# lgen-sudo/EgoM2P

Measured on NVIDIA B200. Metric: ego-b mod4 train nominal tokens/sec (whole job), higher is better.
Workload: dtype bf16

## Files before the change

### egom2p_b200/_lib.py

```python
from __future__ import annotations

import ctypes as C
import os

_HERE = os.path.dirname(os.path.abspath(__file__))
LIB_PATH = os.path.join(_HERE, "libegom2p_b200.so")
MAX_MODS = 8

vp, i32, i64, f32 = C.c_void_p, C.c_int32, C.c_int64, C.c_float


class PlanDesc(C.Structure):
    _fields_ = [("n_mods", i32), ("batch", i32), ("budget", i32), ("is_decoder", i32), ("causal", i32), ("sep", i32),
                ("len", i32 * MAX_MODS), ("mod_id", i32 * MAX_MODS), ("mask", vp * MAX_MODS),
                ("attn_cnt", vp * MAX_MODS), ("ids", vp * MAX_MODS)]


class EmbedDesc(C.Structure):
    _fields_ = [("n_mods", i32), ("dim", i32), ("len", i32 * MAX_MODS), ("vocab", i32 * MAX_MODS),
                ("ids", vp * MAX_MODS), ("token_emb", vp * MAX_MODS), ("pos_emb", vp * MAX_MODS),
                ("mod_emb", vp * MAX_MODS)]


SIGNATURES = {
    "egom2p_last_error": [],
    "egom2p_abi_version": [],
    "egom2p_launch_count": [],
    "egom2p_index_plan": [C.POINTER(PlanDesc), vp, vp, vp, vp, vp, vp, vp, vp, vp, vp],
    "egom2p_plan_rows": [vp, i64, C.POINTER(i32), i32, i64, vp, vp, vp],
    "egom2p_embed_gather_fwd": [C.POINTER(EmbedDesc), vp, vp, vp, vp, vp, i64, i32, vp, vp, vp],
    "egom2p_embed_gather_bwd": [C.POINTER(EmbedDesc), vp, vp, vp, vp, vp, vp, i64, i32, vp, vp, vp, vp],
    "egom2p_layernorm_fwd": [vp, vp, i64, i32, f32, vp, vp, vp, vp, vp],
    "egom2p_layernorm_bwd": [vp, vp, vp, vp, vp, vp, vp, i64, i32, vp, vp, vp, vp],
    "egom2p_layernorm_bias_fwd": [vp, vp, vp, i64, i32, f32, vp, vp, vp, vp, vp],
    "egom2p_layernorm_bias_bwd": [vp, vp, vp, vp, vp, vp, vp, i64, i32, vp, vp, vp, vp, vp],
    "egom2p_gemm_bf16": [vp, vp, i32, i32, i32, i64, i64, i32, i32, vp, vp, i64, vp, vp, i64, vp],
    "egom2p_gemm_swiglu_fwd": [vp, vp, i32, i32, i32, i64, i64, vp, i64, vp, i64, vp],
    "egom2p_gemm_swiglu_bwd": [vp, vp, vp, i32, i32, i32, i64, i64, i64, vp, i64, vp],
    "egom2p_gemm_gelu_fwd": [vp, vp, vp, i32, i32, i32, i64, i64, vp, i64, vp, i64, vp],
    "egom2p_gemm_gelu_bwd": [vp, vp, vp, i32, i32, i32, i64, i64, i64, vp, i64, vp],
    "egom2p_ce_partials": [vp, vp, vp, i32, i32, i32, i64, i64, vp, vp, vp, vp],
    "egom2p_ce_finalize": [vp, vp, vp, i32, i32, vp, vp, vp],
    "egom2p_ce_dlogits": [vp, vp, vp, vp, vp, i32, i32, i32, i32, i64, i64, vp, i64, vp],
    "egom2p_attn_lse_stride": [i32],
    "egom2p_attn_ranges_bytes": [i32, i32],
    "egom2p_attn_ranges": [vp, vp, i32, i32, i32, f32, i32, vp, vp],
    "egom2p_attn_fwd": [vp, vp, vp, i32, i32, i32, i32, i64, i64, i64, vp, vp, i64, vp, vp, vp],
    "egom2p_attn_bwd_scratch_bytes": [i32, i32, i32],
    "egom2p_attn_bwd": [vp, vp, vp, vp, vp, vp, i32, i32, i32, i32, i64, i64, i64, i64, vp, f32, vp, vp, vp, vp,
                        i64, i64, i64, vp],
    "egom2p_cast_f32_to_bf16": [vp, vp, i64, vp],
    "egom2p_cast_f32_to_bf16_multi": [vp, i32, i64, vp],
    "egom2p_add_f32": [vp, vp, i64, vp, vp, vp],
    "egom2p_sumsq_multi": [vp, i32, i64, vp, vp, vp],
    "egom2p_adamw_multi_steps": [vp, i32, i64, f32, f32, f32, vp, vp, f32, vp],
    "egom2p_image_masks": [vp, C.c_uint64, C.c_uint64, i32, i32, i32, vp, vp, vp, vp, vp, vp],
    "egom2p_sample_rows": [vp, i64, i32, i32, f32, f32, i32, vp, vp, vp, vp, vp],
    "egom2p_cfg_combine_bf16": [vp, vp, i64, f32, vp, vp],
    "egom2p_colsum_f32": [vp, i64, i32, vp, vp],
    "egom2p_colsum_bf16": [vp, i64, i32, i64, vp, vp],
    "egom2p_gather_rows_bf16": [vp, vp, i64, i32, vp, vp],
    "egom2p_scatter_rows_f32": [vp, vp, i64, i32, vp, vp],
}
_RESTYPES = {"egom2p_last_error": C.c_char_p, "egom2p_launch_count": i64, "egom2p_attn_bwd_scratch_bytes": i64, "egom2p_attn_ranges_bytes": i64}

_lib = None


def load() -> C.CDLL:
    global _lib
    if _lib is None:
        if not os.path.exists(LIB_PATH):
            raise RuntimeError(f"{LIB_PATH} not found: the CUDA library is mandatory (no fallback path). "
                               "Run `python -m egom2p_b200.build`.")
        lib = C.CDLL(LIB_PATH)
        for name, args in SIGNATURES.items():
            fn = getattr(lib, name)
            fn.argtypes = args
            fn.restype = _RESTYPES.get(name, C.c_int)
        _lib = lib
    return _lib


def check(rc: int, what: str = "") -> None:
    if rc != 0:
        msg = load().egom2p_last_error()
        raise RuntimeError(f"egom2p_b200 {what} failed (code {rc}): {msg.decode() if msg else '?'}")


def launch_count() -> int:
    return int(load().egom2p_launch_count())
```

### egom2p_b200/csrc/attn_bwd.cu

```cuda
#include "attn_common.cuh"

namespace egom2p {

constexpr int kBwdMathWarps = 8;
constexpr int kBwdThreads = 32 * (kBwdMathWarps + 7);
constexpr int kDrainWarp0 = kBwdMathWarps, kBwdTmaWarp = kBwdMathWarps + 4, kBwdMmaWarp = kBwdMathWarps + 5,
              kBwdMmaWarpB = kBwdMathWarps + 6;
constexpr int kBwdStages = 3;
constexpr int kBwdMetaBytes = 5 * kT * 4;
constexpr int kMaxQBlocks = 1024;

struct BwdParams {
  int B, H, Mq, Nk, S;
  RangeMeta meta;
  const float* lse2;
  const float* ndelta;
  float scale_log2;
  uint16_t* dK;
  uint16_t* dV;
  int64_t lddk, lddv;
  int tma_out;
};
struct BwdSmem {
  static constexpr int kTile = kT * 128;
  static constexpr int kK = 0, kV = kK + kTile, kQ = kV + kTile, kDO = kQ + kBwdStages * kTile,
                       kDS = kDO + kBwdStages * kTile,
                       kBox = kDS + 2 * kTile,
                       kMeta = kBox + 8 * 4096, kList = kMeta + kBwdStages * kBwdMetaBytes,
                       kBar = kList + kMaxQBlocks * 2, kTotal = kBar + 256 + 1024;
};
static_assert(BwdSmem::kTotal <= 232448, "attention backward exceeds the 227 KB shared memory of one CTA");


#ifdef EGOM2P_TRACE
__device__ long long g_trace[16 * 64];
#define TRACE(slot, idx)                                                                          \
  do {                                                                                            \
    if (blockIdx.x == 0 && blockIdx.y == 0 && blockIdx.z == gridDim.z - 1 && (idx) < 64 && (threadIdx.x & 31) == 0) \
      g_trace[(slot) * 64 + (idx)] = clock64();                                                   \
  } while (0)
#else
#define TRACE(slot, idx) do {} while (0)
#endif

__device__ __forceinline__ void tmem_st32(uint32_t taddr, const uint32_t (&r)[32]) {
  asm volatile(
      "tcgen05.st.sync.aligned.32x32b.x32.b32 [%0], "
      "{%1, %2, %3, %4, %5, %6, %7, %8, %9, %10, %11, %12, %13, %14, %15, %16, "
      "%17, %18, %19, %20, %21, %22, %23, %24, %25, %26, %27, %28, %29, %30, %31, %32};"
      ::"r"(taddr), "r"(r[0]), "r"(r[1]), "r"(r[2]), "r"(r[3]), "r"(r[4]), "r"(r[5]), "r"(r[6]), "r"(r[7]), "r"(r[8]),
        "r"(r[9]), "r"(r[10]), "r"(r[11]), "r"(r[12]), "r"(r[13]), "r"(r[14]), "r"(r[15]), "r"(r[16]), "r"(r[17]),
        "r"(r[18]), "r"(r[19]), "r"(r[20]), "r"(r[21]), "r"(r[22]), "r"(r[23]), "r"(r[24]), "r"(r[25]), "r"(r[26]),
        "r"(r[27]), "r"(r[28]), "r"(r[29]), "r"(r[30]), "r"(r[31])
      : "memory");
}
__device__ __forceinline__ void tmem_st16(uint32_t taddr, const uint32_t (&r)[16]) {
  asm volatile(
      "tcgen05.st.sync.aligned.32x32b.x16.b32 [%0], "
      "{%1, %2, %3, %4, %5, %6, %7, %8, %9, %10, %11, %12, %13, %14, %15, %16};"
      ::"r"(taddr), "r"(r[0]), "r"(r[1]), "r"(r[2]), "r"(r[3]), "r"(r[4]), "r"(r[5]), "r"(r[6]), "r"(r[7]), "r"(r[8]),
        "r"(r[9]), "r"(r[10]), "r"(r[11]), "r"(r[12]), "r"(r[13]), "r"(r[14]), "r"(r[15])
      : "memory");
}
__device__ __forceinline__ void tmem_st_wait() { asm volatile("tcgen05.wait::st.sync.aligned;" ::: "memory"); }
__device__ __forceinline__ float4 lds_f4(const void* p) {
  float4 v;
  asm volatile("ld.shared.v4.f32 {%0, %1, %2, %3}, [%4];" : "=f"(v.x), "=f"(v.y), "=f"(v.z), "=f"(v.w) : "r"(smem_u32(p)));
  return v;
}

__global__ void __launch_bounds__(kBwdThreads, 1)
attn_bwd_kernel(const __grid_constant__ CUtensorMap tmQ, const __grid_constant__ CUtensorMap tmDO,
                const __grid_constant__ CUtensorMap tmK, const __grid_constant__ CUtensorMap tmV,
                const __grid_constant__ CUtensorMap tmDQ, const __grid_constant__ CUtensorMap tmDK,
                const __grid_constant__ CUtensorMap tmDV, const BwdParams p) {
  extern __shared__ uint8_t smem_raw[];
  uint8_t* smem = reinterpret_cast<uint8_t*>((reinterpret_cast<uintptr_t>(smem_raw) + 1023) & ~(uintptr_t)1023);
  uint8_t *sK = smem + BwdSmem::kK, *sV = smem + BwdSmem::kV, *sQ = smem + BwdSmem::kQ, *sDO = smem + BwdSmem::kDO,
          *sDS = smem + BwdSmem::kDS, *sBox = smem + BwdSmem::kBox, *sMeta = smem + BwdSmem::kMeta;
  uint16_t* s_list = reinterpret_cast<uint16_t*>(smem + BwdSmem::kList);
  uint64_t* bars = reinterpret_cast<uint64_t*>(smem + BwdSmem::kBar);
  uint64_t* kv_full = bars;
  uint64_t* q_full = bars + 1;
  uint64_t* q_empty = q_full + kBwdStages;
  uint64_t* s_full = q_empty + kBwdStages;
  uint64_t* s_free = s_full + 1;
  uint64_t* dp_full = s_free + 1;
  uint64_t* dp_free = dp_full + 1;
  uint64_t* p_full = dp_free + 1;
  uint64_t* p_empty = p_full + 1;
  uint64_t* ds_full = p_empty + 1;
  uint64_t* ds_empty = ds_full + 1;
  uint64_t* dq_full = ds_empty + 1;
  uint64_t* dq_free = dq_full + 1;
  uint64_t* dkv_full = dq_free + 1;
  uint64_t* kv_tmem = dkv_full + 1;
  uint32_t* tmem_slot = reinterpret_cast<uint32_t*>(kv_tmem + 1);
  int* s_n = reinterpret_cast<int*>(tmem_slot + 1);

  const int warp = threadIdx.x >> 5, lane = threadIdx.x & 31;
  const int kv0 = blockIdx.x * kT, h = blockIdx.y, b = blockIdx.z;
  const int nqb = p.S / kT;
  if (warp == 0) TRACE(5, 63);
  if (warp == kDrainWarp0 && lane == 0) {
    tma_prefetch_desc(&tmQ);
    tma_prefetch_desc(&tmDO);
    tma_prefetch_desc(&tmDQ);
    tma_prefetch_desc(&tmDK);
    tma_prefetch_desc(&tmDV);
  }
  if (warp == kBwdTmaWarp && lane == 0) {
    mbar_init(kv_full, 1);
    fence_mbar_init();
    mbar_expect_tx(kv_full, 2 * BwdSmem::kTile);
    tma_load_2d(sK, &tmK, kv_full, h * kD, b * p.Nk + kv0);
    tma_load_2d(sV, &tmV, kv_full, h * kD, b * p.Nk + kv0);
    for (int i = 0; i < kBwdStages; ++i) { mbar_init(&q_full[i], 1); mbar_init(&q_empty[i], 1); }
    mbar_init(s_full, 1);   mbar_init(s_free, kBwdMathWarps);
    mbar_init(dp_full, 1);  mbar_init(dp_free, 1);
    mbar_init(p_full, kBwdMathWarps);  mbar_init(p_empty, 1);
    mbar_init(ds_full, kBwdMathWarps); mbar_init(ds_empty, 1);
    mbar_init(dq_full, 1);  mbar_init(dq_free, 4);
    mbar_init(dkv_full, 1);
    mbar_init(kv_tmem, kBwdMathWarps);
    fence_mbar_init();
    TRACE(5, 57);
  }
  auto issue_q_block = [&](int qblk, int st) {
    const int r0 = qblk * kT;
    uint8_t* meta = sMeta + st * kBwdMetaBytes;
    const int64_t hoff = ((int64_t)b * p.H + h) * p.S + r0, roff = (int64_t)b * p.S + r0;
    mbar_expect_tx(&q_full[st], 2 * BwdSmem::kTile + kBwdMetaBytes);
    tma_load_2d(sQ + st * BwdSmem::kTile, &tmQ, &q_full[st], h * kD, b * p.Mq + r0);
    tma_load_2d(sDO + st * BwdSmem::kTile, &tmDO, &q_full[st], h * kD, b * p.Mq + r0);
    bulk_load(meta + 0 * 512, p.lse2 + hoff, 512, &q_full[st]);
    bulk_load(meta + 1 * 512, p.ndelta + hoff, 512, &q_full[st]);
    bulk_load(meta + 2 * 512, p.meta.row_lo + roff, 512, &q_full[st]);
    bulk_load(meta + 3 * 512, p.meta.row_hi + roff, 512, &q_full[st]);
    bulk_load(meta + 4 * 512, p.meta.row_scale + roff, 512, &q_full[st]);
  };
  if (warp == kBwdTmaWarp) {
    int first = -1;
    for (int i0 = 0; i0 < nqb && first < 0; i0 += 32) {
      const int i = i0 + lane;
      bool take = false;
      if (i < nqb) {
        const int64_t o = ((int64_t)b * nqb + i) * 2;
        const int lo = min(p.meta.blk_lo[o], p.meta.blk_lo[o + 1]), hi = max(p.meta.blk_hi[o], p.meta.blk_hi[o + 1]);
        take = hi > kv0 && lo < kv0 + kT;
      }
      const unsigned msk = __ballot_sync(0xffffffffu, take);
      if (msk) first = i0 + __ffs(msk) - 1;
    }
    __syncwarp();
    if (first >= 0 && lane == 0) issue_q_block(first, 0);
  }
  if (warp == 0) {
    int n = 0;
    for (int i0 = 0; i0 < nqb; i0 += 32) {
      const int i = i0 + lane;
      bool take = false, inside = false, normal = false;
      if (i < nqb) {
        const int64_t o = ((int64_t)b * nqb + i) * 2;
        const int lo = min(p.meta.blk_lo[o], p.meta.blk_lo[o + 1]), hi = max(p.meta.blk_hi[o], p.meta.blk_hi[o + 1]);
        take = hi > kv0 && lo < kv0 + kT;
        inside = max(p.meta.blk_lo_max[o], p.meta.blk_lo_max[o + 1]) <= kv0 &&
                 min(p.meta.blk_hi_min[o], p.meta.blk_hi_min[o + 1]) >= kv0 + kT;
        normal = p.meta.blk_lo_max[o] != INT_MAX && p.meta.blk_lo_max[o + 1] != INT_MAX;
      }
      const unsigned msk = __ballot_sync(0xffffffffu, take);
      const int pos = n + __popc(msk & ((1u << lane) - 1));
      if (take && pos < kMaxQBlocks) s_list[pos] = (uint16_t)(i | (inside ? 0x8000 : 0) | (normal ? 0x4000 : 0));
      n += __popc(msk);
    }
    if (lane == 0) *s_n = n < kMaxQBlocks ? n : kMaxQBlocks;
    TRACE(5, 55);
  }
  if (warp == kBwdMmaWarp) {
    tmem_alloc<512>(tmem_slot);
    TRACE(5, 54);
  }
  if (warp == 1) TRACE(5, 53);
  tc_fence_before();
  __syncthreads();
  tc_fence_after();
  const uint32_t tmem_base = *tmem_slot;
  const int n = *s_n;
  if (warp == 0) TRACE(5, 62);
  constexpr uint32_t cS = 0, cDP = 128, cDV = 256, cDK = 320, cDQ = 384, cK = 448, cV = 480;

  if (warp >= kBwdTmaWarp) {
    if (warp == kBwdTmaWarp) {
      if (n == 0) mbar_wait(kv_full, 0);
      if (n > 0) {
        for (int idx = 1; idx < n; ++idx) {
          const int st = idx % kBwdStages;
          mbar_wait(&q_empty[st], ((idx / kBwdStages) & 1) ^ 1);
          if (elect_one()) issue_q_block((int)(s_list[idx] & 0x3fff), st);
          __syncwarp();
        }
      }
    } else if (warp == kBwdMmaWarp) {
      if (n > 0) {
        constexpr uint32_t idesc_kk = umma_idesc_bf16(128, kT, 0, 0);
        constexpr uint32_t idesc_tm = umma_idesc_bf16(128, kD, 0, 1);
        constexpr uint32_t idesc_mm = umma_idesc_bf16(128, kD, 1, 1);
        const uint32_t tS = tmem_base + cS, tDP = tmem_base + cDP, tDQ = tmem_base + cDQ, tK = tmem_base + cK, tV = tmem_base + cV;
        const uint64_t dKm0 = umma_desc_mnmajor_sw128(smem_u32(sK), 8192);
        const uint64_t dDSm0 = umma_desc_mnmajor_sw128(smem_u32(sDS), BwdSmem::kTile);
        auto issue_s = [&](int st) {
          const uint64_t dQ0 = umma_desc_kmajor_sw128(smem_u32(sQ + st * BwdSmem::kTile));
          if (elect_one()) {
#pragma unroll
            for (int k = 0; k < 4; ++k) umma_bf16_ts(tS, tK + 8 * k, dQ0 + 2 * k, idesc_kk, k ? 1u : 0u);
            umma_commit(s_full);
          }
          __syncwarp();
        };
        auto issue_dp = [&](int st) {
          const uint64_t dDO0 = umma_desc_kmajor_sw128(smem_u32(sDO + st * BwdSmem::kTile));
          if (elect_one()) {
#pragma unroll
            for (int k = 0; k < 4; ++k) umma_bf16_ts(tDP, tV + 8 * k, dDO0 + 2 * k, idesc_kk, k ? 1u : 0u);
            umma_commit(dp_full);
          }
          __syncwarp();
        };
        mbar_wait(kv_tmem, 0);
        mbar_wait(&q_full[0], 0);
        tc_fence_after();
        issue_s(0);
        issue_dp(0);
        for (int idx = 0; idx < n; ++idx) {
          const int st1 = (idx + 1) % kBwdStages;
          const uint32_t par = idx & 1;
          if (idx + 1 < n) {
            mbar_wait(&q_full[st1], ((idx + 1) / kBwdStages) & 1);
            mbar_wait(s_free, par);
            mbar_wait(p_empty, par);
            tc_fence_after();
            TRACE(0, idx);
            issue_s(st1);
          }
          mbar_wait(ds_full, par);
          if (idx > 0) mbar_wait(dq_free, (idx - 1) & 1);
          tc_fence_after();
          TRACE(4, idx);
          if (elect_one()) {
#pragma unroll
            for (int k = 0; k < 8; ++k) umma_bf16_ss(tDQ, dDSm0 + 128 * k, dKm0 + 128 * k, idesc_mm, k ? 1u : 0u);
            umma_commit(dq_full);
            umma_commit(ds_empty);
          }
          __syncwarp();
          if (idx + 1 < n) {
            mbar_wait(dp_free, par);
            tc_fence_after();
            TRACE(2, idx);
            issue_dp(st1);
          }
        }
      }
    } else if (warp == kBwdMmaWarpB) {
      if (n > 0) {
        constexpr uint32_t idesc_tm = umma_idesc_bf16(128, kD, 0, 1);
        const uint32_t tS = tmem_base + cS, tDP = tmem_base + cDP, tDV = tmem_base + cDV, tDK = tmem_base + cDK;
        for (int idx = 0; idx < n; ++idx) {
          const int st = idx % kBwdStages;
          const uint32_t par = idx & 1;
          mbar_wait(p_full, par);
          tc_fence_after();
          TRACE(1, idx);
          const uint64_t dDOm0 = umma_desc_mnmajor_sw128(smem_u32(sDO + st * BwdSmem::kTile), 8192);
          if (elect_one()) {
#pragma unroll
            for (int k = 0; k < 8; ++k)
              umma_bf16_ts(tDV, tS + (k < 4 ? 8 * k : 64 + 8 * (k - 4)), dDOm0 + 128 * k, idesc_tm, (idx | k) ? 1u : 0u);
            umma_commit(p_empty);
          }
          __syncwarp();
          mbar_wait(ds_full, par);
          tc_fence_after();
          TRACE(3, idx);
          const uint64_t dQm0 = umma_desc_mnmajor_sw128(smem_u32(sQ + st * BwdSmem::kTile), 8192);
          if (elect_one()) {
#pragma unroll
            for (int k = 0; k < 8; ++k)
              umma_bf16_ts(tDK, tDP + (k < 4 ? 8 * k : 64 + 8 * (k - 4)), dQm0 + 128 * k, idesc_tm, (idx | k) ? 1u : 0u);
            umma_commit(&q_empty[st]);
            umma_commit(dp_free);
            if (idx == n - 1) umma_commit(dkv_full);
          }
          __syncwarp();
        }
      }
    }
  } else if (warp >= kDrainWarp0) {
    const int quarter = warp & 3;
    uint8_t* box0 = sBox + quarter * 8192;
    const uint32_t t_dq = tmem_base + ((uint32_t)(quarter * 32) << 16) + cDQ;
    for (int idx = 0; idx < n; ++idx) {
      const int r0 = (int)(s_list[idx] & 0x3fff) * kT + quarter * 32;
      mbar_wait(dq_full, idx & 1);
      tc_fence_after();
      if (warp == kDrainWarp0) TRACE(11, idx);
      const bool live = r0 < p.Mq;
      if (lane == 0) tma_store_wait_read();
      __syncwarp();
#pragma unroll
      for (int hb = 0; hb < 2; ++hb) {
        uint32_t v[32];
        uint8_t* box = box0 + hb * 4096;
        tmem_ld32(t_dq + hb * 32, v);
        tmem_ld_wait();
        if (hb == 1) {
          tc_fence_before();
          __syncwarp();
          if (lane == 0) mbar_arrive(dq_free);
        }
        if (live) {
#pragma unroll
          for (int j = 0; j < 8; ++j)
            *reinterpret_cast<uint4*>(box + lane * 128 + ((j ^ (lane & 7)) << 4)) = make_uint4(v[4 * j], v[4 * j + 1], v[4 * j + 2], v[4 * j + 3]);
          fence_async_smem();
          __syncwarp();
          if (lane == 0) {
            tma_reduce_add_2d(&tmDQ, box, h * kD + hb * 32, b * p.Mq + r0);
            tma_store_commit();
          }
        }
      }
      if (warp == kDrainWarp0) TRACE(12, idx);
    }
    if (lane == 0) tma_store_wait_read();
  } else {
    const int quarter = warp & 3, half = warp >> 2;
    const int trow = quarter * 32 + lane;
    const int kidx = kv0 + trow;
    const uint32_t t_lane = tmem_base + ((uint32_t)(quarter * 32) << 16);
    uint8_t* pDS = sDS + half * BwdSmem::kTile;
    const float SC = p.scale_log2, RN = p.scale_log2 * kLn2;
    if (n > 0) {
      mbar_wait(kv_full, 0);
      if (warp == 0) TRACE(5, 56);
      uint32_t kw[16], vw[16];
#pragma unroll
      for (int c = 0; c < 4; ++c) {
        const uint4 a = *reinterpret_cast<const uint4*>(sK + swz_off(trow, half * 4 + c));
        const uint4 d = *reinterpret_cast<const uint4*>(sV + swz_off(trow, half * 4 + c));
        kw[4 * c] = a.x; kw[4 * c + 1] = a.y; kw[4 * c + 2] = a.z; kw[4 * c + 3] = a.w;
        vw[4 * c] = d.x; vw[4 * c + 1] = d.y; vw[4 * c + 2] = d.z; vw[4 * c + 3] = d.w;
      }
      tmem_st16(t_lane + cK + half * 16, kw);
      tmem_st16(t_lane + cV + half * 16, vw);
      tmem_st_wait();
      tc_fence_before();
      __syncwarp();
      if (lane == 0) mbar_arrive(kv_tmem);
      if (warp == 0) TRACE(5, 58);
    }
    for (int idx = 0; idx < n; ++idx) {
      const int st = idx % kBwdStages;
      const uint32_t par = idx & 1;
      const bool inside = (s_list[idx] & 0x8000) != 0, normal = (s_list[idx] & 0x4000) != 0;
      const float* m_ls = reinterpret_cast<const float*>(sMeta + st * kBwdMetaBytes) + half * 64;
      const float* m_nd = m_ls + kT;
      const int* m_lo = reinterpret_cast<const int*>(m_ls + 2 * kT);
      const int* m_hi = m_lo + kT;
      const float* m_rs = m_ls + 4 * kT;
      uint32_t pp[32];
      {
        uint32_t s0[32], s1[32];
        if (warp == 0) TRACE(5, idx);
        mbar_wait(&q_full[st], (idx / kBwdStages) & 1);
        mbar_wait(s_full, par);
        tc_fence_after();
        if (warp == 0) TRACE(6, idx);
        tmem_ld32(t_lane + cS + half * 64, s0);
        tmem_ld32(t_lane + cS + half * 64 + 32, s1);
        tmem_ld_wait();
        tc_fence_before();
        __syncwarp();
        if (lane == 0) mbar_arrive(s_free);
        if (inside) {
#pragma unroll
          for (int c4 = 0; c4 < 8; ++c4) {
            const float4 la = lds_f4(m_ls + 4 * c4), lb = lds_f4(m_ls + 32 + 4 * c4);
            s0[4 * c4] = __float_as_uint(fmaf(__uint_as_float(s0[4 * c4]), SC, -la.x));
            s0[4 * c4 + 1] = __float_as_uint(fmaf(__uint_as_float(s0[4 * c4 + 1]), SC, -la.y));
            s0[4 * c4 + 2] = __float_as_uint(fmaf(__uint_as_float(s0[4 * c4 + 2]), SC, -la.z));
            s0[4 * c4 + 3] = __float_as_uint(fmaf(__uint_as_float(s0[4 * c4 + 3]), SC, -la.w));
            s1[4 * c4] = __float_as_uint(fmaf(__uint_as_float(s1[4 * c4]), SC, -lb.x));
            s1[4 * c4 + 1] = __float_as_uint(fmaf(__uint_as_float(s1[4 * c4 + 1]), SC, -lb.y));
            s1[4 * c4 + 2] = __float_as_uint(fmaf(__uint_as_float(s1[4 * c4 + 2]), SC, -lb.z));
            s1[4 * c4 + 3] = __float_as_uint(fmaf(__uint_as_float(s1[4 * c4 + 3]), SC, -lb.w));
          }
#pragma unroll
          for (int c = 0; c < 32; ++c) {
            s0[c] = __float_as_uint((c & 3) == 3 ? ex2_poly(__uint_as_float(s0[c])) : ex2(__uint_as_float(s0[c])));
            s1[c] = __float_as_uint((c & 3) == 3 ? ex2_poly(__uint_as_float(s1[c])) : ex2(__uint_as_float(s1[c])));
          }
#pragma unroll
          for (int c = 0; c < 16; ++c) {
            pp[c] = pack_bf16(__uint_as_float(s0[2 * c]), __uint_as_float(s0[2 * c + 1]));
            pp[16 + c] = pack_bf16(__uint_as_float(s1[2 * c]), __uint_as_float(s1[2 * c + 1]));
          }
        } else if (normal) {
#pragma unroll
          for (int c4 = 0; c4 < 8; ++c4) {
#pragma unroll
            for (int g = 0; g < 2; ++g) {
              uint32_t(&sv)[32] = g ? s1 : s0;
              const float4 l = lds_f4(m_ls + g * 32 + 4 * c4), lo = lds_f4(m_lo + g * 32 + 4 * c4), hi = lds_f4(m_hi + g * 32 + 4 * c4);
              const float lv[4] = {l.x, l.y, l.z, l.w};
              const int lov[4] = {__float_as_int(lo.x), __float_as_int(lo.y), __float_as_int(lo.z), __float_as_int(lo.w)};
              const int hiv[4] = {__float_as_int(hi.x), __float_as_int(hi.y), __float_as_int(hi.z), __float_as_int(hi.w)};
#pragma unroll
              for (int u = 0; u < 4; ++u) {
                const bool ok = kidx >= lov[u] && kidx < hiv[u];
                sv[4 * c4 + u] = ok ? __float_as_uint(fmaf(__uint_as_float(sv[4 * c4 + u]), SC, -lv[u])) : 0xff800000u;
              }
            }
          }
#pragma unroll
          for (int c = 0; c < 32; ++c) {
            s0[c] = __float_as_uint(ex2(__uint_as_float(s0[c])));
            s1[c] = __float_as_uint(ex2(__uint_as_float(s1[c])));
          }
#pragma unroll
          for (int c = 0; c < 16; ++c) {
            pp[c] = pack_bf16(__uint_as_float(s0[2 * c]), __uint_as_float(s0[2 * c + 1]));
            pp[16 + c] = pack_bf16(__uint_as_float(s1[2 * c]), __uint_as_float(s1[2 * c + 1]));
          }
        } else {
#pragma unroll
          for (int c = 0; c < 32; ++c) {
            float e[2];
#pragma unroll
            for (int u = 0; u < 2; ++u) {
              const int q = 2 * c + u;
              const float rs = m_rs[q];
              const bool ok = kidx >= m_lo[q] && kidx < m_hi[q];
              const float sv = __uint_as_float(q < 32 ? s0[q & 31] : s1[q & 31]);
              e[u] = ok ? ex2(fmaf(rs != 0.f ? sv : 0.f, rs, -m_ls[q])) : 0.f;
            }
            pp[c] = pack_bf16(e[0], e[1]);
          }
        }
      }
      if (warp == 0) TRACE(7, idx);
      tmem_st32(t_lane + cS + half * 64, pp);
      uint32_t d0[32];
      mbar_wait(dp_full, par);
      tc_fence_after();
      tmem_ld32(t_lane + cDP + half * 64, d0);
      tmem_st_wait();
      tc_fence_before();
      __syncwarp();
      if (lane == 0) mbar_arrive(p_full);
      if (warp == 0) TRACE(8, idx);
      auto dsmul = [&](const uint32_t (&d)[32], int hh) {
        if (inside || normal) {
#pragma unroll
          for (int c4 = 0; c4 < 8; ++c4) {
            const float4 nd = lds_f4(m_nd + hh * 32 + 4 * c4);
            const uint32_t t0 = pack_bf16(fmaf(__uint_as_float(d[4 * c4]), RN, nd.x), fmaf(__uint_as_float(d[4 * c4 + 1]), RN, nd.y));
            const uint32_t t1 = pack_bf16(fmaf(__uint_as_float(d[4 * c4 + 2]), RN, nd.z), fmaf(__uint_as_float(d[4 * c4 + 3]), RN, nd.w));
            asm("mul.rn.bf16x2 %0, %1, %2;" : "=r"(pp[hh * 16 + 2 * c4]) : "r"(pp[hh * 16 + 2 * c4]), "r"(t0));
            asm("mul.rn.bf16x2 %0, %1, %2;" : "=r"(pp[hh * 16 + 2 * c4 + 1]) : "r"(pp[hh * 16 + 2 * c4 + 1]), "r"(t1));
          }
        } else {
#pragma unroll
          for (int c4 = 0; c4 < 8; ++c4) {
            const float4 nd = lds_f4(m_nd + hh * 32 + 4 * c4);
            const float4 rs = lds_f4(m_rs + hh * 32 + 4 * c4);
            const uint32_t t0 = pack_bf16(fmaf(__uint_as_float(d[4 * c4]), rs.x * kLn2, nd.x), fmaf(__uint_as_float(d[4 * c4 + 1]), rs.y * kLn2, nd.y));
            const uint32_t t1 = pack_bf16(fmaf(__uint_as_float(d[4 * c4 + 2]), rs.z * kLn2, nd.z), fmaf(__uint_as_float(d[4 * c4 + 3]), rs.w * kLn2, nd.w));
            asm("mul.rn.bf16x2 %0, %1, %2;" : "=r"(pp[hh * 16 + 2 * c4]) : "r"(pp[hh * 16 + 2 * c4]), "r"(t0));
            asm("mul.rn.bf16x2 %0, %1, %2;" : "=r"(pp[hh * 16 + 2 * c4 + 1]) : "r"(pp[hh * 16 + 2 * c4 + 1]), "r"(t1));
          }
        }
      };
      tmem_ld_wait();
      if (warp == 0) TRACE(9, idx);
      dsmul(d0, 0);
      if (warp == 0) TRACE(13, idx);
      tmem_ld32(t_lane + cDP + half * 64 + 32, d0);
      if (idx > 0) mbar_wait(ds_empty, (idx - 1) & 1);
      tmem_ld_wait();
      if (warp == 0) TRACE(14, idx);
      dsmul(d0, 1);
      if (warp == 0) TRACE(15, idx);
      tmem_st32(t_lane + cDP + half * 64, pp);
#pragma unroll
      for (int c8 = 0; c8 < 8; ++c8)
        *reinterpret_cast<uint4*>(pDS + swz_off(trow, c8)) = make_uint4(pp[4 * c8], pp[4 * c8 + 1], pp[4 * c8 + 2], pp[4 * c8 + 3]);
      fence_async_smem();
      tmem_st_wait();
      tc_fence_before();
      __syncwarp();
      if (lane == 0) mbar_arrive(ds_full);
      if (warp == 0) TRACE(10, idx);
    }
    if (n > 0) {
      mbar_wait(dkv_full, 0);
      tc_fence_after();
    }
    if (warp == 0) TRACE(5, 61);
#pragma unroll 1
    for (int which = 0; which < 2; ++which) {
      uint32_t v[32];
      if (n > 0) {
        tmem_ld32(t_lane + (which == 0 ? cDV : cDK) + half * 32, v);
        tmem_ld_wait();
      } else {
#pragma unroll
        for (int c = 0; c < 32; ++c) v[c] = 0u;
      }
      uint4 pk[4];
#pragma unroll
      for (int c8 = 0; c8 < 4; ++c8) {
        pk[c8].x = pack_bf16(__uint_as_float(v[c8 * 8 + 0]), __uint_as_float(v[c8 * 8 + 1]));
        pk[c8].y = pack_bf16(__uint_as_float(v[c8 * 8 + 2]), __uint_as_float(v[c8 * 8 + 3]));
        pk[c8].z = pack_bf16(__uint_as_float(v[c8 * 8 + 4]), __uint_as_float(v[c8 * 8 + 5]));
        pk[c8].w = pack_bf16(__uint_as_float(v[c8 * 8 + 6]), __uint_as_float(v[c8 * 8 + 7]));
      }
      if (p.tma_out) {
        uint8_t* stage = which == 0 ? sQ : sDO;
#pragma unroll
        for (int c8 = 0; c8 < 4; ++c8) *reinterpret_cast<uint4*>(stage + swz_off(trow, half * 4 + c8)) = pk[c8];
        if (warp == 0) TRACE(5, 52 - which);
      } else if (kidx < p.Nk) {
        uint16_t* out = (which == 0 ? p.dV + ((int64_t)b * p.Nk + kidx) * p.lddv : p.dK + ((int64_t)b * p.Nk + kidx) * p.lddk) +
                        h * kD + half * 32;
#pragma unroll
        for (int c8 = 0; c8 < 4; ++c8) reinterpret_cast<uint4*>(out)[c8] = pk[c8];
      }
    }
    if (p.tma_out) {
      fence_async_smem();
      asm volatile("bar.sync 1, 256;" ::: "memory");
      if (warp == 0) TRACE(5, 50);
      if (warp == 0 && lane == 0) {
        tma_store_2d(&tmDV, sQ, h * kD, b * p.Nk + kv0);
        tma_store_2d(&tmDK, sDO, h * kD, b * p.Nk + kv0);
        tma_store_commit();
        tma_store_wait_read();
      }
    }
    if (warp == 0) TRACE(5, 60);
  }
  tc_fence_before();
  __syncthreads();
  if (warp == 0) TRACE(5, 59);
  if (warp == kBwdMmaWarp) {
    tc_fence_after();
    tmem_dealloc<512>(tmem_base);
  }
}

__global__ void __launch_bounds__(256) attn_bwd_prep_kernel(const uint16_t* __restrict__ O, const uint16_t* __restrict__ dO,
                                                            int64_t ldo, const float* __restrict__ row_scale, int B, int H,
                                                            int Mq, int S, float* __restrict__ ndelta, float* __restrict__ dq_acc) {
  const int64_t wid = (int64_t)blockIdx.x * 8 + (threadIdx.x >> 5);
  const int lane = threadIdx.x & 31;
  if (wid >= (int64_t)B * S) return;
  const int b = (int)(wid / S), r = (int)(wid % S);
  if (r >= Mq) {
    for (int hh = lane; hh < H; hh += 32) ndelta[((int64_t)b * H + hh) * S + r] = 0.f;
    return;
  }
  const float rs = row_scale[wid] * kLn2;
  const uint16_t* po = O + ((int64_t)b * Mq + r) * ldo;
  const uint16_t* pd = dO + ((int64_t)b * Mq + r) * ldo;
  float4* acc = reinterpret_cast<float4*>(dq_acc + ((int64_t)b * Mq + r) * (int64_t)H * kD);
  const int chunks = H * 8;
  for (int c0 = 0; c0 < chunks; c0 += 32) {
    const int c = c0 + lane;
    float part = 0.f;
    if (c < chunks) {
      const uint4 a = reinterpret_cast<const uint4*>(po)[c], g = reinterpret_cast<const uint4*>(pd)[c];
      const uint32_t aw[4] = {a.x, a.y, a.z, a.w}, gw[4] = {g.x, g.y, g.z, g.w};
#pragma unroll
      for (int u = 0; u < 4; ++u) {
        const float2 fa = __bfloat1622float2(*reinterpret_cast<const __nv_bfloat162*>(&aw[u]));
        const float2 fg = __bfloat1622float2(*reinterpret_cast<const __nv_bfloat162*>(&gw[u]));
        part += fa.x * fg.x + fa.y * fg.y;
      }
      acc[2 * c] = make_float4(0.f, 0.f, 0.f, 0.f);
      acc[2 * c + 1] = make_float4(0.f, 0.f, 0.f, 0.f);
    }
    part += __shfl_xor_sync(0xffffffffu, part, 1);
    part += __shfl_xor_sync(0xffffffffu, part, 2);
    part += __shfl_xor_sync(0xffffffffu, part, 4);
    if (c < chunks && (lane & 7) == 0) ndelta[((int64_t)b * H + (c >> 3)) * S + r] = -part * rs;
  }
}

__global__ void __launch_bounds__(256) attn_bwd_dq_cast_kernel(const float* __restrict__ acc, int64_t rows, int cols8,
                                                               uint16_t* __restrict__ dq, int64_t lddq) {
  const int64_t total = rows * cols8;
  for (int64_t i = (int64_t)blockIdx.x * blockDim.x + threadIdx.x; i < total; i += (int64_t)gridDim.x * blockDim.x) {
    const int64_t r = i / cols8;
    const int c = (int)(i % cols8);
    const float4 a = reinterpret_cast<const float4*>(acc + r * cols8 * 8)[2 * c];
    const float4 g = reinterpret_cast<const float4*>(acc + r * cols8 * 8)[2 * c + 1];
    uint4 pk;
    pk.x = pack_bf16(a.x, a.y); pk.y = pack_bf16(a.z, a.w); pk.z = pack_bf16(g.x, g.y); pk.w = pack_bf16(g.z, g.w);
    reinterpret_cast<uint4*>(dq + r * lddq)[c] = pk;
  }
}

}

#ifdef EGOM2P_TRACE
extern "C" int egom2p_debug_attn_trace(long long* host_dst) {
  return (int)cudaMemcpyFromSymbol(host_dst, egom2p::g_trace, sizeof(egom2p::g_trace));
}
#endif

extern "C" int64_t egom2p_attn_bwd_scratch_bytes(int32_t B, int32_t H, int32_t Mq) {
  using namespace egom2p;
  return align256((int64_t)B * H * padS(Mq) * 4) + align256((int64_t)B * Mq * H * kD * 4) + 256;
}

extern "C" int egom2p_attn_bwd(const uint16_t* Q, const uint16_t* K, const uint16_t* V, const uint16_t* O, const uint16_t* dO,
                               const float* lse, int32_t B, int32_t H, int32_t Mq, int32_t Nk, int64_t ldq, int64_t ldk,
                               int64_t ldv, int64_t ldo, const void* meta, float scale, void* scratch, uint16_t* dQ,
                               uint16_t* dK, uint16_t* dV, int64_t lddq, int64_t lddk, int64_t lddv, void* stream_) {
  using namespace egom2p;
  cudaStream_t stream = (cudaStream_t)stream_;
  EGO_REQUIRE(Q && O && dO && lse && meta && scratch && dQ && B > 0 && H > 0 && Mq > 0 && Nk >= 0, "attn_bwd: bad argument");
  EGO_REQUIRE(((uintptr_t)scratch & 255) == 0 && ((uintptr_t)lse & 255) == 0 && ((uintptr_t)meta & 255) == 0,
              "attn_bwd: scratch / lse / meta must be 256-byte aligned");
  EGO_REQUIRE(lddq % 8 == 0 && ((uintptr_t)dQ & 15) == 0 && ldo % 8 == 0 && ((uintptr_t)O & 15) == 0 && ((uintptr_t)dO & 15) == 0,
              "attn_bwd: dQ / O / dO alignment");
  const int S = padS(Mq);
  EGO_REQUIRE(S / kT <= kMaxQBlocks, "attn_bwd: Mq too large (max %d)", kMaxQBlocks * kT);
  RangeMeta rm = carve_meta(const_cast<void*>(meta), B, Mq);
  float* ndelta = reinterpret_cast<float*>(scratch);
  float* dq_acc = reinterpret_cast<float*>(reinterpret_cast<char*>(scratch) + align256((int64_t)B * H * S * 4));

  attn_bwd_prep_kernel<<<(unsigned)(((int64_t)B * S + 7) / 8), 256, 0, stream>>>(O, dO, ldo, rm.row_scale, B, H, Mq, S, ndelta, dq_acc);
  int rc = check_launch("attn_bwd prep");
  if (rc) return rc;
  if (Nk > 0) {
    EGO_REQUIRE(K && V && dK && dV, "attn_bwd: K / V / dK / dV missing");
    EGO_REQUIRE(lddk % 8 == 0 && lddv % 8 == 0 && ((uintptr_t)dK & 15) == 0 && ((uintptr_t)dV & 15) == 0, "attn_bwd: dK/dV alignment");
    static std::atomic<uint64_t> attr_done{0};
    if ((rc = ensure_dyn_smem(attn_bwd_kernel, BwdSmem::kTotal, attr_done, "attn_bwd"))) return rc;
    CUtensorMap tmQ, tmDO, tmK, tmV, tmDQ, tmDK, tmDV;
    if ((rc = make_tmap_bf16_2d(&tmQ, Q, (uint64_t)B * Mq, (uint64_t)H * kD, ldq, kT, kD))) return rc;
    if ((rc = make_tmap_bf16_2d(&tmDO, dO, (uint64_t)B * Mq, (uint64_t)H * kD, ldo, kT, kD))) return rc;
    if ((rc = make_tmap_bf16_2d(&tmK, K, (uint64_t)B * Nk, (uint64_t)H * kD, ldk, kT, kD))) return rc;
    if ((rc = make_tmap_bf16_2d(&tmV, V, (uint64_t)B * Nk, (uint64_t)H * kD, ldv, kT, kD))) return rc;
    if ((rc = make_tmap_2d(&tmDQ, dq_acc, 4, (uint64_t)B * Mq, (uint64_t)H * kD, (uint64_t)H * kD, 32, 32))) return rc;
    const int tma_out = (Nk % kT == 0 || B == 1) ? 1 : 0;
    if (tma_out) {
      if ((rc = make_tmap_bf16_2d(&tmDK, dK, (uint64_t)B * Nk, (uint64_t)H * kD, lddk, kT, kD))) return rc;
      if ((rc = make_tmap_bf16_2d(&tmDV, dV, (uint64_t)B * Nk, (uint64_t)H * kD, lddv, kT, kD))) return rc;
    } else {
      tmDK = tmK;
      tmDV = tmV;
    }
    BwdParams pb{B, H, Mq, Nk, S, rm, lse, ndelta, scale * kLog2e, dK, dV, lddk, lddv, tma_out};
    attn_bwd_kernel<<<dim3((Nk + kT - 1) / kT, H, B), kBwdThreads, BwdSmem::kTotal, stream>>>(tmQ, tmDO, tmK, tmV, tmDQ, tmDK, tmDV, pb);
    if ((rc = check_launch("attn_bwd"))) return rc;
  }
  const int64_t rows = (int64_t)B * Mq;
  const int cols8 = H * kD / 8;
  const int64_t total = rows * cols8;
  attn_bwd_dq_cast_kernel<<<(unsigned)((total + 255) / 256 < 148 * 16 ? (total + 255) / 256 : 148 * 16), 256, 0, stream>>>(dq_acc, rows, cols8, dQ, lddq);
  return check_launch("attn_bwd dq cast");
}
```

### egom2p_b200/ops.py

```python
from __future__ import annotations

import ctypes as C
from typing import Dict, Optional, Sequence

import torch

from . import _lib

bf16, f32 = torch.bfloat16, torch.float32


def _s() -> int:
    return torch.cuda.current_stream().cuda_stream


def _req_current(t: torch.Tensor):
    if t.device.index is not None and t.device.index != torch.cuda.current_device():
        raise RuntimeError(f"egom2p_b200: tensor on {t.device} but the current CUDA device is {torch.cuda.current_device()}; "
                           "wrap the call in torch.cuda.device(tensor.device)")


class KernelTimer:
    active: Optional["KernelTimer"] = None

    def __init__(self):
        self.records = []

    def __enter__(self):
        KernelTimer.active = self
        return self

    def __exit__(self, *exc):
        KernelTimer.active = None

    def summary(self):
        torch.cuda.synchronize()
        out: Dict[str, Dict[str, float]] = {}
        for fam, work, unit, e0, e1 in self.records:
            d = out.setdefault(fam, {"ms": 0.0, "work": 0.0, "launches": 0, "unit": unit})
            d["ms"] += e0.elapsed_time(e1)
            d["work"] += float(work)
            d["launches"] += 1
        return out


class _timed:
    __slots__ = ("fam", "work", "unit", "e0")

    def __init__(self, fam: str, work: float, unit: str):
        self.fam, self.work, self.unit = fam, work, unit

    def __enter__(self):
        if KernelTimer.active is not None:
            self.e0 = torch.cuda.Event(enable_timing=True)
            self.e0.record()

    def __exit__(self, *exc):
        t = KernelTimer.active
        if t is not None:
            e1 = torch.cuda.Event(enable_timing=True)
            e1.record()
            t.records.append((self.fam, self.work, self.unit, self.e0, e1))


def _p(t: Optional[torch.Tensor]):
    return None if t is None else t.data_ptr()


def _req(t: torch.Tensor, dtype, name: str):
    if not t.is_cuda:
        raise RuntimeError(f"egom2p_b200: {name} must be a CUDA tensor (no CPU fallback exists)")
    if t.dtype != dtype:
        raise TypeError(f"egom2p_b200: {name} must be {dtype}, got {t.dtype}")
    _req_current(t)
    return t


class Plan:
    __slots__ = ("keep_idx", "keep_mod", "keep_pos", "pad", "mod_mask", "n_valid", "target_ids", "key_lo", "key_hi",
                 "B", "budget", "order", "row_batch", "rows", "slot_index", "slot_to_row")

    def __init__(self):
        self.row_batch = None
        self.rows = None


def index_plan(masks: Sequence[torch.Tensor], mod_ids: Sequence[int], budget: int, *, decoder: bool = False,
               attn_cnt: Optional[Sequence[torch.Tensor]] = None, ids: Optional[Sequence[torch.Tensor]] = None,
               causal: bool = False, sep: bool = True) -> Plan:
    lib = _lib.load()
    B = masks[0].shape[0]
    dev = masks[0].device
    d = _lib.PlanDesc()
    d.n_mods, d.batch, d.is_decoder, d.causal, d.sep = len(masks), B, int(decoder), int(causal), int(sep)
    keep = []
    total = 0
    for i, m in enumerate(masks):
        m = _req(m.reshape(B, -1), torch.bool, "mask").contiguous()
        keep.append(m)
        d.len[i], d.mod_id[i], d.mask[i] = m.shape[1], int(mod_ids[i]), m.data_ptr()
        total += m.shape[1]
        if decoder:
            a = _req(attn_cnt[i].reshape(B, -1), torch.int32, "decoder_attention_mask").contiguous()
            t = _req(ids[i].reshape(B, -1), torch.int64, "ids").contiguous()
            keep += [a, t]
            d.attn_cnt[i], d.ids[i] = a.data_ptr(), t.data_ptr()
    budget = min(int(budget), total)
    d.budget = budget
    pl = Plan()
    pl.B, pl.budget = B, budget
    pl.keep_idx = torch.empty(B, budget, dtype=torch.int32, device=dev)
    pl.keep_mod = torch.empty_like(pl.keep_idx)
    pl.keep_pos = torch.empty_like(pl.keep_idx)
    pl.pad = torch.empty(B, budget, dtype=torch.bool, device=dev)
    pl.mod_mask = torch.empty(B, budget, dtype=torch.int16, device=dev)
    pl.n_valid = torch.empty(B, dtype=torch.int32, device=dev)
    pl.target_ids = pl.key_lo = pl.key_hi = None
    if decoder:
        pl.target_ids = torch.empty(B, budget, dtype=torch.int64, device=dev)
        pl.key_lo = torch.empty(B, budget, dtype=torch.int32, device=dev)
        pl.key_hi = torch.empty_like(pl.key_lo)
    _lib.check(lib.egom2p_index_plan(C.byref(d), _p(pl.keep_idx), _p(pl.keep_mod), _p(pl.keep_pos), _p(pl.pad),
                                     _p(pl.mod_mask), _p(pl.n_valid), _p(pl.target_ids), _p(pl.key_lo), _p(pl.key_hi),
                                     _s()), "index_plan")
    return pl


def plan_rows(mod_mask: torch.Tensor, mod_ids: Sequence[int]):
    lib = _lib.load()
    _req(mod_mask, torch.int16, "mod_mask")
    flat = mod_mask.reshape(-1).contiguous()
    total, n = flat.numel(), len(mod_ids)
    rows = torch.empty(n, total, dtype=torch.int64, device=flat.device)
    counts = torch.empty(n, dtype=torch.int32, device=flat.device)
    ids = (C.c_int32 * n)(*[int(i) for i in mod_ids])
    _lib.check(lib.egom2p_plan_rows(_p(flat), total, ids, n, total, _p(rows), _p(counts), _s()), "plan_rows")
    return rows, counts


def _embed_desc(dim, lens, vocabs, ids, tables, pos, mod):
    d = _lib.EmbedDesc()
    d.n_mods, d.dim = len(lens), dim
    for i in range(len(lens)):
        d.len[i], d.vocab[i] = lens[i], vocabs[i]
        d.ids[i] = _p(ids[i]) if ids is not None else None
        d.token_emb[i] = _p(tables[i]) if tables is not None else None
        d.pos_emb[i], d.mod_emb[i] = _p(pos[i]), _p(mod[i])
    return d


def embed_gather_fwd(plan: Plan, dim: int, lens, vocabs, ids, tables, pos, mod, mask_token=None, want_emb=True):
    lib = _lib.load()
    packed = plan.rows is not None
    rows = plan.rows if packed else plan.B * plan.budget
    dev = plan.keep_mod.device
    x0 = torch.empty((rows, dim) if packed else (plan.B, plan.budget, dim), dtype=f32, device=dev)
    emb = torch.empty_like(x0) if want_emb else None
    d = _embed_desc(dim, lens, vocabs, ids, tables, pos, mod)
    with _timed("embed_gather", rows * dim * 4.0 * (2 + (1 if mask_token is None else 0) + (1 if want_emb else 0)), "byte"):
        _lib.check(lib.egom2p_embed_gather_fwd(C.byref(d), _p(mask_token), _p(plan.keep_mod), _p(plan.keep_pos), _p(plan.pad),
                                               _p(plan.row_batch), rows, plan.budget, _p(x0), _p(emb), _s()), "embed_gather_fwd")
    return x0, emb


def embed_gather_bwd(plan: Plan, dim: int, lens, vocabs, ids, pos, mod, dx0, demb, d_tables, d_mod, d_mask_token):
    lib = _lib.load()
    rows = plan.rows if plan.rows is not None else plan.B * plan.budget
    d = _embed_desc(dim, lens, vocabs, ids, None, pos, mod)
    n = len(lens)
    arr_t = (C.c_void_p * _lib.MAX_MODS)(*[(_p(t) if t is not None else None) for t in (d_tables or [None] * n)])
    arr_m = (C.c_void_p * _lib.MAX_MODS)(*[(_p(t) if t is not None else None) for t in (d_mod or [None] * n)])
    _lib.check(lib.egom2p_embed_gather_bwd(C.byref(d), _p(dx0), _p(demb), _p(plan.keep_mod), _p(plan.keep_pos),
                                           _p(plan.pad), _p(plan.row_batch), rows, plan.budget, C.cast(arr_t, C.c_void_p),
                                           C.cast(arr_m, C.c_void_p), _p(d_mask_token), _s()), "embed_gather_bwd")


def layernorm_fwd(x: torch.Tensor, w: torch.Tensor, eps: float = 1e-6, out_bf16=True, out_f32=False, save_stats=True, bias=None):
    lib = _lib.load()
    _req(x, f32, "x"); _req(w, f32, "weight")
    D = x.shape[-1]
    rows = x.numel() // D
    yb = torch.empty(x.shape, dtype=bf16, device=x.device) if out_bf16 else None
    yf = torch.empty_like(x) if out_f32 else None
    mean = torch.empty(rows, dtype=f32, device=x.device) if save_stats else None
    rstd = torch.empty(rows, dtype=f32, device=x.device) if save_stats else None
    with _timed("layernorm_fwd", rows * D * (4.0 + (2 if out_bf16 else 0) + (4 if out_f32 else 0)), "byte"):
        if bias is None:
            _lib.check(lib.egom2p_layernorm_fwd(_p(x), _p(w), rows, D, eps, _p(yb), _p(yf), _p(mean), _p(rstd), _s()), "layernorm_fwd")
        else:
            _req(bias, f32, "bias")
            _lib.check(lib.egom2p_layernorm_bias_fwd(_p(x), _p(w), _p(bias), rows, D, eps, _p(yb), _p(yf), _p(mean), _p(rstd), _s()),
                       "layernorm_bias_fwd")
    return yb, yf, mean, rstd


def layernorm_bwd(dy: torch.Tensor, x, w, mean, rstd, dx_in=None, d_weight=None, want_bf16=False, d_bias=None):
    lib = _lib.load()
    D = x.shape[-1]
    rows = x.numel() // D
    dx = torch.empty_like(x)
    dxb = torch.empty(x.shape, dtype=bf16, device=x.device) if want_bf16 else None
    dyb = dy if dy.dtype == bf16 else None
    dyf = dy if dy.dtype == f32 else None
    nbytes = rows * D * (4.0 + dy.element_size() + 4 + (4 if dx_in is not None else 0) + (2 if want_bf16 else 0))
    with _timed("layernorm_bwd", nbytes, "byte"):
        if d_bias is None:
            _lib.check(lib.egom2p_layernorm_bwd(_p(dyb), _p(dyf), _p(x), _p(w), _p(mean), _p(rstd), _p(dx_in), rows, D, _p(dx),
                                                _p(dxb), _p(d_weight), _s()), "layernorm_bwd")
        else:
            _req(d_bias, f32, "d_bias")
            _lib.check(lib.egom2p_layernorm_bias_bwd(_p(dyb), _p(dyf), _p(x), _p(w), _p(mean), _p(rstd), _p(dx_in), rows, D,
                                                     _p(dx), _p(dxb), _p(d_weight), _p(d_bias), _s()), "layernorm_bias_bwd")
    return dx, dxb


def gemm(A: torch.Tensor, B: torch.Tensor, M: int, N: int, K: int, *, a_mn=False, b_mn=False, bias=None, addend=None,
         out_bf16: Optional[torch.Tensor] = None, out_f32: Optional[torch.Tensor] = None):
    lib = _lib.load()
    _req(A, bf16, "A"); _req(B, bf16, "B")
    assert A.dim() == 2 and B.dim() == 2 and A.stride(1) == 1 and B.stride(1) == 1
    out = out_bf16 if out_bf16 is not None else out_f32
    assert out is not None and out.stride(-1) == 1
    ldc = out.stride(0)
    if out_bf16 is not None and out_f32 is not None:
        assert out_bf16.stride(0) == out_f32.stride(0)
    with _timed("gemm", 2.0 * M * N * K, "flop"):
        _lib.check(lib.egom2p_gemm_bf16(_p(A), _p(B), M, N, K, A.stride(0), B.stride(0), int(a_mn), int(b_mn), _p(bias),
                                        _p(addend), addend.stride(0) if addend is not None else 0, _p(out_bf16), _p(out_f32),
                                        ldc, _s()), "gemm_bf16")
    return out


def gemm_swiglu_fwd(x: torch.Tensor, w13: torch.Tensor):
    lib = _lib.load()
    R, K = x.shape
    N2 = w13.shape[0]
    ab = torch.empty(R, N2, dtype=bf16, device=x.device)
    g = torch.empty(R, N2 // 2, dtype=bf16, device=x.device)
    with _timed("gemm", 2.0 * R * N2 * K, "flop"):
        _lib.check(lib.egom2p_gemm_swiglu_fwd(_p(x), _p(w13), R, N2, K, x.stride(0), w13.stride(0), _p(ab), ab.stride(0), _p(g),
                                              g.stride(0), _s()), "gemm_swiglu_fwd")
    return ab, g


def gemm_swiglu_bwd(dy: torch.Tensor, w2: torch.Tensor, ab: torch.Tensor):
    lib = _lib.load()
    R, K = dy.shape
    hidden = w2.shape[1]
    dab = torch.empty(R, 2 * hidden, dtype=bf16, device=dy.device)
    with _timed("gemm", 2.0 * R * hidden * K, "flop"):
        _lib.check(lib.egom2p_gemm_swiglu_bwd(_p(dy), _p(w2), _p(ab), R, hidden, K, dy.stride(0), w2.stride(0), ab.stride(0),
                                              _p(dab), dab.stride(0), _s()), "gemm_swiglu_bwd")
    return dab


def gemm_gelu_fwd(x: torch.Tensor, w1: torch.Tensor, b1: Optional[torch.Tensor]):
    lib = _lib.load()
    R, K = x.shape
    N = w1.shape[0]
    if b1 is not None:
        _req(b1, f32, "b1")
    u = torch.empty(R, N, dtype=bf16, device=x.device)
    h = torch.empty(R, N, dtype=bf16, device=x.device)
    with _timed("gemm", 2.0 * R * N * K, "flop"):
        _lib.check(lib.egom2p_gemm_gelu_fwd(_p(x), _p(w1), _p(b1), R, N, K, x.stride(0), w1.stride(0), _p(u), u.stride(0), _p(h),
                                            h.stride(0), _s()), "gemm_gelu_fwd")
    return u, h


def gemm_gelu_bwd(dy: torch.Tensor, w2: torch.Tensor, u: torch.Tensor):
    lib = _lib.load()
    R, K = dy.shape
    hidden = w2.shape[1]
    du = torch.empty(R, hidden, dtype=bf16, device=dy.device)
    with _timed("gemm", 2.0 * R * hidden * K, "flop"):
        _lib.check(lib.egom2p_gemm_gelu_bwd(_p(dy), _p(w2), _p(u), R, hidden, K, dy.stride(0), w2.stride(0), u.stride(0), _p(du),
                                            du.stride(0), _s()), "gemm_gelu_bwd")
    return du


def linear_fwd(x: torch.Tensor, w: torch.Tensor, *, bias=None, addend=None, out_dtype=bf16):
    R, K = x.shape
    N = w.shape[0]
    y = torch.empty(R, N, dtype=out_dtype, device=x.device)
    gemm(x, w, R, N, K, bias=bias, addend=addend, out_bf16=y if out_dtype == bf16 else None,
         out_f32=y if out_dtype == f32 else None)
    return y


def linear_dgrad(dy: torch.Tensor, w: torch.Tensor, *, addend=None, out_dtype=bf16):
    R, N = dy.shape
    K = w.shape[1]
    dx = torch.empty(R, K, dtype=out_dtype, device=dy.device)
    gemm(dy, w, R, K, N, b_mn=True, addend=addend, out_bf16=dx if out_dtype == bf16 else None,
         out_f32=dx if out_dtype == f32 else None)
    return dx


def linear_wgrad(dy: torch.Tensor, x: torch.Tensor, out: Optional[torch.Tensor] = None, accumulate=False):
    R, N = dy.shape
    K = x.shape[1]
    if out is None:
        out = torch.empty(N, K, dtype=f32, device=dy.device)
    gemm(dy, x, N, K, R, a_mn=True, b_mn=True, addend=out if accumulate else None, out_f32=out)
    return out


def ce_forward(y: torch.Tensor, w: torch.Tensor, target: torch.Tensor):
    lib = _lib.load()
    R, K = y.shape
    V = w.shape[0]
    nt = 2 * ((V + 255) // 256)
    dev = y.device
    pm = torch.empty(nt, R, dtype=f32, device=dev)
    ps = torch.empty(nt, R, dtype=f32, device=dev)
    tl = torch.zeros(R, dtype=f32, device=dev)
    lse = torch.empty(R, dtype=f32, device=dev)
    loss = torch.zeros(1, dtype=f32, device=dev)
    with _timed("head_ce", 2.0 * R * V * K, "flop"):
        _lib.check(lib.egom2p_ce_partials(_p(y), _p(w), _p(target), R, V, K, y.stride(0), w.stride(0), _p(pm), _p(ps), _p(tl),
                                          _s()), "ce_partials")
    _lib.check(lib.egom2p_ce_finalize(_p(pm), _p(ps), _p(tl), R, nt, _p(lse), _p(loss), _s()), "ce_finalize")
    return loss, lse


def ce_dlogits(y, w, target, lse, gscale: torch.Tensor, v0: int, vc: int, out: torch.Tensor):
    lib = _lib.load()
    R, K = y.shape
    with _timed("head_ce", 2.0 * R * vc * K, "flop"):
        _lib.check(lib.egom2p_ce_dlogits(_p(y), _p(w), _p(target), _p(lse), _p(gscale), R, v0, vc, K, y.stride(0), w.stride(0),
                                         _p(out), out.stride(0), _s()), "ce_dlogits")
    return out


def lse_stride(Mq: int) -> int:
    return int(_lib.load().egom2p_attn_lse_stride(Mq))


def attn_ranges(B, Mq, Nk, key_lo=None, key_hi=None, scale=None, device=None, empty_zero=False):
    lib = _lib.load()
    scale = (64 ** -0.5) if scale is None else scale
    device = device if device is not None else key_lo.device
    meta = torch.empty(lib.egom2p_attn_ranges_bytes(B, Mq), dtype=torch.uint8, device=device)
    _lib.check(lib.egom2p_attn_ranges(_p(key_lo), _p(key_hi), B, Mq, Nk, scale, int(empty_zero), _p(meta), _s()), "attn_ranges")
    return meta


def attn_fwd(q, k, v, B, H, Mq, Nk, key_lo=None, key_hi=None, scale=None, want_lse=True, meta=None, pairs=None):
    lib = _lib.load()
    if meta is None:
        meta = attn_ranges(B, Mq, Nk, key_lo, key_hi, scale, device=q.device)
    o = torch.empty(B * Mq, H * 64, dtype=bf16, device=q.device)
    lse = torch.empty(B, H, lse_stride(Mq), dtype=f32, device=q.device) if want_lse else None
    kmax = torch.empty(B * H, dtype=f32, device=q.device) if Nk > 0 else None
    with _timed("attn_fwd", 4.0 * H * 64 * (pairs if pairs is not None else B * Mq * Nk), "flop"):
        _lib.check(lib.egom2p_attn_fwd(_p(q), _p(k) if Nk > 0 else None, _p(v) if Nk > 0 else None, B, H, Mq, Nk, q.stride(0),
                                       k.stride(0) if Nk > 0 else 0, v.stride(0) if Nk > 0 else 0, _p(meta), _p(o),
                                       o.stride(0), _p(lse), _p(kmax), _s()), "attn_fwd")
    return o, lse


def attn_bwd(q, k, v, o, do, lse, B, H, Mq, Nk, dq, dk, dv, key_lo=None, key_hi=None, scale=None, meta=None, pairs=None):
    lib = _lib.load()
    scale = (64 ** -0.5) if scale is None else scale
    if meta is None:
        meta = attn_ranges(B, Mq, Nk, key_lo, key_hi, scale, device=q.device)
    assert do.stride(0) == o.stride(0)
    scratch = torch.empty(lib.egom2p_attn_bwd_scratch_bytes(B, H, Mq), dtype=torch.uint8, device=q.device)
    with _timed("attn_bwd", 10.0 * H * 64 * (pairs if pairs is not None else B * Mq * Nk), "flop"):
        _lib.check(lib.egom2p_attn_bwd(_p(q), _p(k), _p(v), _p(o), _p(do), _p(lse), B, H, Mq, Nk, q.stride(0), k.stride(0),
                                       v.stride(0), o.stride(0), _p(meta), scale, _p(scratch), _p(dq), _p(dk), _p(dv),
                                       dq.stride(0), dk.stride(0), dv.stride(0), _s()), "attn_bwd")


def cast_bf16(src: torch.Tensor, out: Optional[torch.Tensor] = None):
    lib = _lib.load()
    _req(src, f32, "src")
    src = src.contiguous()
    if out is None:
        out = torch.empty(src.shape, dtype=bf16, device=src.device)
    with _timed("cast", src.numel() * 6.0, "byte"):
        _lib.check(lib.egom2p_cast_f32_to_bf16(_p(src), _p(out), src.numel(), _s()), "cast_f32_to_bf16")
    return out


GRAD_GEN = [0]
_OPERAND_CACHE: Dict[int, tuple] = {}


def cached_bf16(weight: torch.Tensor) -> torch.Tensor:
    w = weight.detach()
    key = id(weight)
    sig = (w.data_ptr(), weight._version, GRAD_GEN[0], tuple(w.shape))
    hit = _OPERAND_CACHE.get(key)
    if hit is not None and hit[0] == sig:
        return hit[1]
    wb = cast_bf16(w.contiguous())
    if len(_OPERAND_CACHE) > 64:
        _OPERAND_CACHE.clear()
    _OPERAND_CACHE[key] = (sig, wb)
    return wb


class CastPlan:

    def __init__(self, items):
        import numpy as np
        dt = np.dtype([("src", "<u8"), ("dst", "<u8"), ("rows", "<i8"), ("first_chunk", "<i8"), ("cols", "<i4"), ("dst_ld", "<i4"),
                       ("group", "<i4"), ("slot", "<i4"), ("rows_per_chunk", "<i4"), ("pad", "<i4")])
        assert dt.itemsize == 56
        tab = np.zeros(len(items), dtype=dt)
        chunk = 0
        self.bytes = 0.0
        self.ptrs = []
        for i, (src, dst, group, slot) in enumerate(items):
            _req(src, f32, "src"); _req(dst, bf16, "dst")
            assert src.dim() == 2 and src.is_contiguous() and dst.dim() == 2 and dst.stride(1) == 1
            rows, cols = src.shape
            need_rows = rows if group == 0 else (rows + group - 1) // group * 2 * group
            assert dst.shape[0] >= need_rows and dst.shape[1] >= cols, "cast plan: destination too small"
            rpc = max(1, 8192 // cols)
            tab[i] = (src.data_ptr(), dst.data_ptr(), rows, chunk, cols, dst.stride(0), group, slot, rpc, 0)
            chunk += (rows + rpc - 1) // rpc
            self.bytes += rows * cols * 6.0
            self.ptrs.append((src.data_ptr(), dst.data_ptr()))
        self.n_items, self.n_chunks = len(items), chunk
        self.table = torch.from_numpy(tab.view(np.uint8).reshape(-1).copy()).to(items[0][0].device)

    def run(self):
        lib = _lib.load()
        with _timed("cast", self.bytes, "byte"):
            _lib.check(lib.egom2p_cast_f32_to_bf16_multi(_p(self.table), self.n_items, self.n_chunks, _s()), "cast_f32_to_bf16_multi")


def add_f32(a, b, want_f32=True, want_bf16=False):
    lib = _lib.load()
    out = torch.empty_like(a) if want_f32 else None
    outb = torch.empty(a.shape, dtype=bf16, device=a.device) if want_bf16 else None
    _lib.check(lib.egom2p_add_f32(_p(a), _p(b), a.numel(), _p(out), _p(outb), _s()), "add_f32")
    return out, outb


def colsum(x: torch.Tensor, out: torch.Tensor):
    lib = _lib.load()
    rows, cols = x.shape
    _lib.check(lib.egom2p_colsum_f32(_p(x), rows, cols, _p(out), _s()), "colsum_f32")
    return out


def colsum_bf16(x: torch.Tensor, out: Optional[torch.Tensor] = None):
    lib = _lib.load()
    _req(x, bf16, "x")
    assert x.dim() == 2 and x.stride(1) == 1
    rows, cols = x.shape
    if out is None:
        out = torch.zeros(cols, dtype=f32, device=x.device)
    if rows:
        with _timed("bias_grad", rows * cols * 2.0, "byte"):
            _lib.check(lib.egom2p_colsum_bf16(_p(x), rows, cols, x.stride(0), _p(out), _s()), "colsum_bf16")
    return out


def gather_rows_bf16(src: torch.Tensor, idx: torch.Tensor):
    lib = _lib.load()
    n, cols = idx.numel(), src.shape[1]
    dst = torch.empty(n, cols, dtype=bf16, device=src.device)
    if n:
        _lib.check(lib.egom2p_gather_rows_bf16(_p(src), _p(idx), n, cols, _p(dst), _s()), "gather_rows_bf16")
    return dst


def scatter_rows_f32(src: torch.Tensor, idx: torch.Tensor, dst: torch.Tensor):
    lib = _lib.load()
    n, cols = idx.numel(), src.shape[1]
    if n:
        _lib.check(lib.egom2p_scatter_rows_f32(_p(src), _p(idx), n, cols, _p(dst), _s()), "scatter_rows_f32")
    return dst


def sample_rows(logits: torch.Tensor, temperature: float, top_p: float = 0.0, top_k: int = 0, u: Optional[torch.Tensor] = None,
                want_prob: bool = True, want_kept: bool = False):
    lib = _lib.load()
    _req(logits, f32, "logits")
    assert logits.dim() == 2 and logits.stride(1) == 1
    rows, V = logits.shape
    if u is None:
        u = torch.rand(rows, device=logits.device, dtype=f32)
    _req(u, f32, "u")
    tok = torch.empty(rows, dtype=torch.int64, device=logits.device)
    prob = torch.empty(rows, dtype=f32, device=logits.device) if want_prob else None
    kept = torch.empty(rows, dtype=torch.int32, device=logits.device) if want_kept else None
    if rows:
        with _timed("sample", rows * V * 4.0, "byte"):
            _lib.check(lib.egom2p_sample_rows(_p(logits), logits.stride(0), rows, V, float(temperature), float(top_p), int(top_k),
                                              _p(u.contiguous()), _p(tok), _p(prob), _p(kept), _s()), "sample_rows")
    return tok, prob, kept


def cfg_combine_bf16(y_uncond: torch.Tensor, y_cond: torch.Tensor, scale: float) -> torch.Tensor:
    lib = _lib.load()
    _req(y_uncond, f32, "y_uncond"); _req(y_cond, f32, "y_cond")
    assert y_uncond.shape == y_cond.shape and y_uncond.is_contiguous() and y_cond.is_contiguous()
    out = torch.empty(y_uncond.shape, dtype=bf16, device=y_uncond.device)
    if out.numel():
        _lib.check(lib.egom2p_cfg_combine_bf16(_p(y_uncond), _p(y_cond), y_uncond.numel(), float(scale), _p(out), _s()), "cfg_combine_bf16")
    return out
```

### include/egom2p_b200.h

```cpp
#ifndef EGOM2P_B200_H_
#define EGOM2P_B200_H_
#include <stdint.h>

#ifdef __cplusplus
extern "C" {
#endif

#define EGOM2P_OK 0
#define EGOM2P_ERR_INVALID (-1)
#define EGOM2P_ERR_CUDA (-2)

#define EGOM2P_MAX_MODS 8

const char* egom2p_last_error(void);
int egom2p_abi_version(void);
int64_t egom2p_launch_count(void);

typedef struct {
  int32_t n_mods;
  int32_t batch;
  int32_t budget;
  int32_t is_decoder;
  int32_t causal;
  int32_t sep;
  int32_t len[EGOM2P_MAX_MODS];
  int32_t mod_id[EGOM2P_MAX_MODS];
  const uint8_t* mask[EGOM2P_MAX_MODS];
  const int32_t* attn_cnt[EGOM2P_MAX_MODS];
  const int64_t* ids[EGOM2P_MAX_MODS];
} egom2p_plan_desc;

int egom2p_index_plan(const egom2p_plan_desc* desc, int32_t* keep_idx, int32_t* keep_mod, int32_t* keep_pos,
                      uint8_t* pad, int16_t* mod_mask, int32_t* n_valid, int64_t* target_ids, int32_t* key_lo,
                      int32_t* key_hi, void* stream);

int egom2p_plan_rows(const int16_t* mod_mask, int64_t total, const int32_t* mod_ids, int32_t n_mods, int64_t cap,
                     int64_t* rows, int32_t* counts, void* stream);

typedef struct {
  int32_t n_mods;
  int32_t dim;
  int32_t len[EGOM2P_MAX_MODS];
  int32_t vocab[EGOM2P_MAX_MODS];
  const int64_t* ids[EGOM2P_MAX_MODS];
  const float* token_emb[EGOM2P_MAX_MODS];
  const float* pos_emb[EGOM2P_MAX_MODS];
  const float* mod_emb[EGOM2P_MAX_MODS];
} egom2p_embed_desc;

int egom2p_embed_gather_fwd(const egom2p_embed_desc* desc, const float* mask_token, const int32_t* keep_mod,
                            const int32_t* keep_pos, const uint8_t* pad, const int32_t* row_batch, int64_t rows,
                            int32_t budget, float* x0, float* emb, void* stream);
int egom2p_embed_gather_bwd(const egom2p_embed_desc* desc, const float* dx0, const float* demb, const int32_t* keep_mod,
                            const int32_t* keep_pos, const uint8_t* pad, const int32_t* row_batch, int64_t rows, int32_t budget,
                            float* const* d_token_emb, float* const* d_mod_emb, float* d_mask_token, void* stream);

int egom2p_layernorm_fwd(const float* x, const float* weight, int64_t rows, int32_t dim, float eps, uint16_t* y_bf16,
                         float* y_f32, float* mean, float* rstd, void* stream);
int egom2p_layernorm_bwd(const uint16_t* dy_bf16, const float* dy_f32, const float* x, const float* weight,
                         const float* mean, const float* rstd, const float* dx_in, int64_t rows, int32_t dim,
                         float* dx_out, uint16_t* dx_bf16, float* d_weight, void* stream);
int egom2p_layernorm_bias_fwd(const float* x, const float* weight, const float* bias, int64_t rows, int32_t dim, float eps,
                              uint16_t* y_bf16, float* y_f32, float* mean, float* rstd, void* stream);
int egom2p_layernorm_bias_bwd(const uint16_t* dy_bf16, const float* dy_f32, const float* x, const float* weight,
                              const float* mean, const float* rstd, const float* dx_in, int64_t rows, int32_t dim,
                              float* dx_out, uint16_t* dx_bf16, float* d_weight, float* d_bias, void* stream);

int egom2p_gemm_bf16(const uint16_t* A, const uint16_t* B, int32_t M, int32_t N, int32_t K, int64_t lda, int64_t ldb,
                     int32_t a_mn, int32_t b_mn, const float* bias, const float* addend, int64_t ld_add,
                     uint16_t* c_bf16, float* c_f32, int64_t ldc, void* stream);

int egom2p_gemm_swiglu_fwd(const uint16_t* X, const uint16_t* W13, int32_t M, int32_t N2, int32_t K, int64_t ldx, int64_t ldw,
                           uint16_t* ab, int64_t ld_ab, uint16_t* g, int64_t ldg, void* stream);
int egom2p_gemm_swiglu_bwd(const uint16_t* dY, const uint16_t* W2, const uint16_t* ab, int32_t M, int32_t hidden, int32_t K,
                           int64_t ldy, int64_t ldw, int64_t ld_ab, uint16_t* dab, int64_t ld_dab, void* stream);

int egom2p_gemm_gelu_fwd(const uint16_t* X, const uint16_t* W1, const float* b1, int32_t M, int32_t N, int32_t K, int64_t ldx,
                         int64_t ldw, uint16_t* u, int64_t ld_u, uint16_t* h, int64_t ldh, void* stream);
int egom2p_gemm_gelu_bwd(const uint16_t* dY, const uint16_t* W2, const uint16_t* u, int32_t M, int32_t hidden, int32_t K,
                         int64_t ldy, int64_t ldw, int64_t ld_u, uint16_t* du, int64_t ld_du, void* stream);

int egom2p_ce_partials(const uint16_t* Y, const uint16_t* W, const int64_t* target, int32_t R, int32_t V, int32_t K,
                       int64_t ldy, int64_t ldw, float* part_max, float* part_sum, float* tgt_logit, void* stream);
int egom2p_ce_finalize(const float* part_max, const float* part_sum, const float* tgt_logit, int32_t R,
                       int32_t n_tiles, float* lse, float* loss_sum, void* stream);
int egom2p_ce_dlogits(const uint16_t* Y, const uint16_t* W, const int64_t* target, const float* lse,
                      const float* gscale, int32_t R, int32_t v0, int32_t Vc, int32_t K, int64_t ldy, int64_t ldw,
                      uint16_t* dlogits, int64_t ldd, void* stream);

int egom2p_attn_lse_stride(int32_t Mq);
int64_t egom2p_attn_ranges_bytes(int32_t B, int32_t Mq);
int egom2p_attn_ranges(const int32_t* key_lo, const int32_t* key_hi, int32_t B, int32_t Mq, int32_t Nk, float scale,
                       int32_t empty_zero, void* meta, void* stream);
int egom2p_attn_fwd(const uint16_t* Q, const uint16_t* K, const uint16_t* V, int32_t B, int32_t H, int32_t Mq, int32_t Nk,
                    int64_t ldq, int64_t ldk, int64_t ldv, const void* meta, uint16_t* O, int64_t ldo, float* lse,
                    float* kmax_scratch, void* stream);
int64_t egom2p_attn_bwd_scratch_bytes(int32_t B, int32_t H, int32_t Mq);
int egom2p_attn_bwd(const uint16_t* Q, const uint16_t* K, const uint16_t* V, const uint16_t* O, const uint16_t* dO,
                    const float* lse, int32_t B, int32_t H, int32_t Mq, int32_t Nk, int64_t ldq, int64_t ldk, int64_t ldv,
                    int64_t ldo, const void* meta, float scale, void* scratch, uint16_t* dQ, uint16_t* dK, uint16_t* dV,
                    int64_t lddq, int64_t lddk, int64_t lddv, void* stream);

int egom2p_cast_f32_to_bf16(const float* src, uint16_t* dst, int64_t n, void* stream);
typedef struct {
  const float* src;
  uint16_t* dst;
  int64_t rows;
  int64_t first_chunk;
  int32_t cols, dst_ld, group, slot, rows_per_chunk, pad_;
} egom2p_cast_item;
int egom2p_cast_f32_to_bf16_multi(const void* items_dev, int32_t n_items, int64_t n_chunks, void* stream);
int egom2p_add_f32(const float* a, const float* b, int64_t n, float* out, uint16_t* out_bf16, void* stream);
typedef struct {
  float* param;
  const float* grad;
  float* exp_avg;
  float* exp_avg_sq;
  int64_t n;
  int64_t first_chunk;
  float lr, weight_decay;
} egom2p_opt_item;
int egom2p_sumsq_multi(const void* items_dev, int32_t n_items, int64_t n_chunks, float* partials, float* sumsq, void* stream);
int egom2p_adamw_multi_steps(const void* items_dev, int32_t n_items, int64_t n_chunks, float beta1, float beta2, float eps,
                             int32_t* steps, const float* sumsq, float max_norm, void* stream);
int egom2p_colsum_f32(const float* x, int64_t rows, int32_t cols, float* out, void* stream);
int egom2p_colsum_bf16(const uint16_t* x, int64_t rows, int32_t cols, int64_t ld, float* out, void* stream);
int egom2p_gather_rows_bf16(const uint16_t* src, const int64_t* idx, int64_t n, int32_t cols, uint16_t* dst, void* stream);
int egom2p_scatter_rows_f32(const float* src, const int64_t* idx, int64_t n, int32_t cols, float* dst, void* stream);

int egom2p_image_masks(const float* noise, uint64_t seed, uint64_t offset, int32_t stream_id, int32_t B, int32_t L,
                       const int32_t* input_budget, const int32_t* target_budget, uint8_t* input_mask, uint8_t* target_mask,
                       int32_t* attn_cnt, void* stream);

int egom2p_sample_rows(const float* logits, int64_t ld, int32_t rows, int32_t V, float temperature, float top_p,
                       int32_t top_k, const float* u, int64_t* token, float* prob, int32_t* n_kept, void* stream);
int egom2p_cfg_combine_bf16(const float* y_uncond, const float* y_cond, int64_t n, float scale, uint16_t* out, void* stream);

#ifdef __cplusplus
}
#endif
#endif
```

Baseline: 706,100.

## Make attention backward persistent with atomic tile scheduler and double-buffered K

```diff
diff --git a/egom2p_b200/_lib.py b/egom2p_b200/_lib.py
--- a/egom2p_b200/_lib.py
+++ b/egom2p_b200/_lib.py
@@ -48,7 +48,7 @@
     "egom2p_attn_fwd": [vp, vp, vp, i32, i32, i32, i32, i64, i64, i64, vp, vp, i64, vp, vp, vp],
     "egom2p_attn_bwd_scratch_bytes": [i32, i32, i32],
     "egom2p_attn_bwd": [vp, vp, vp, vp, vp, vp, i32, i32, i32, i32, i64, i64, i64, i64, vp, f32, vp, vp, vp, vp,
-                        i64, i64, i64, vp],
+                        i64, i64, i64, vp, i32],
     "egom2p_cast_f32_to_bf16": [vp, vp, i64, vp],
     "egom2p_cast_f32_to_bf16_multi": [vp, i32, i64, vp],
     "egom2p_add_f32": [vp, vp, i64, vp, vp, vp],
diff --git a/egom2p_b200/csrc/attn_bwd.cu b/egom2p_b200/csrc/attn_bwd.cu
--- a/egom2p_b200/csrc/attn_bwd.cu
+++ b/egom2p_b200/csrc/attn_bwd.cu
@@ -12,6 +12,8 @@
 
 struct BwdParams {
   int B, H, Mq, Nk, S;
+  int ntiles, items;
+  unsigned* counter;
   RangeMeta meta;
   const float* lse2;
   const float* ndelta;
@@ -19,15 +21,15 @@
   uint16_t* dK;
   uint16_t* dV;
   int64_t lddk, lddv;
-  int tma_out;
 };
 struct BwdSmem {
   static constexpr int kTile = kT * 128;
-  static constexpr int kK = 0, kV = kK + kTile, kQ = kV + kTile, kDO = kQ + kBwdStages * kTile,
+  static constexpr int kK = 0,
+                       kV = kK + 2 * kTile, kQ = kV + kTile, kDO = kQ + kBwdStages * kTile,
                        kDS = kDO + kBwdStages * kTile,
                        kBox = kDS + 2 * kTile,
                        kMeta = kBox + 8 * 4096, kList = kMeta + kBwdStages * kBwdMetaBytes,
-                       kBar = kList + kMaxQBlocks * 2, kTotal = kBar + 256 + 1024;
+                       kBar = kList + 2 * kMaxQBlocks * 2, kTotal = kBar + 256 + 1024;
 };
 static_assert(BwdSmem::kTotal <= 232448, "attention backward exceeds the 227 KB shared memory of one CTA");
 
@@ -36,11 +38,13 @@
 __device__ long long g_trace[16 * 64];
 #define TRACE(slot, idx)                                                                          \
   do {                                                                                            \
-    if (blockIdx.x == 0 && blockIdx.y == 0 && blockIdx.z == gridDim.z - 1 && (idx) < 64 && (threadIdx.x & 31) == 0) \
+    if (blockIdx.x == 0 && (idx) < 64 && (threadIdx.x & 31) == 0)                                 \
       g_trace[(slot) * 64 + (idx)] = clock64();                                                   \
   } while (0)
+#define TRACE_B(slot, g) do { if ((g) < 48) TRACE(slot, g); } while (0)
 #else
 #define TRACE(slot, idx) do {} while (0)
+#define TRACE_B(slot, g) do {} while (0)
 #endif
 
 __device__ __forceinline__ void tmem_st32(uint32_t taddr, const uint32_t (&r)[32]) {
@@ -69,11 +73,16 @@
   return v;
 }
 
+__device__ __forceinline__ unsigned bwd_claim_item(unsigned* counter) {
+  unsigned v = 0;
+  if ((threadIdx.x & 31) == 0) v = atomicAdd(counter, 1u);
+  return __shfl_sync(0xffffffffu, v, 0);
+}
+
 __global__ void __launch_bounds__(kBwdThreads, 1)
 attn_bwd_kernel(const __grid_constant__ CUtensorMap tmQ, const __grid_constant__ CUtensorMap tmDO,
                 const __grid_constant__ CUtensorMap tmK, const __grid_constant__ CUtensorMap tmV,
-                const __grid_constant__ CUtensorMap tmDQ, const __grid_constant__ CUtensorMap tmDK,
-                const __grid_constant__ CUtensorMap tmDV, const BwdParams p) {
+                const __grid_constant__ CUtensorMap tmDQ, const BwdParams p) {
   extern __shared__ uint8_t smem_raw[];
   uint8_t* smem = reinterpret_cast<uint8_t*>((reinterpret_cast<uintptr_t>(smem_raw) + 1023) & ~(uintptr_t)1023);
   uint8_t *sK = smem + BwdSmem::kK, *sV = smem + BwdSmem::kV, *sQ = smem + BwdSmem::kQ, *sDO = smem + BwdSmem::kDO,
@@ -95,460 +104,555 @@
   uint64_t* dq_free = dq_full + 1;
   uint64_t* dkv_full = dq_free + 1;
   uint64_t* kv_tmem = dkv_full + 1;
-  uint32_t* tmem_slot = reinterpret_cast<uint32_t*>(kv_tmem + 1);
+  uint64_t* dkv_free = kv_tmem + 1;
+  uint64_t* k_free = dkv_free + 1;
+  uint64_t* v_free = k_free + 2;
+  uint64_t* tile_full = v_free + 1;
+  uint64_t* tile_empty = tile_full + 2;
+  uint32_t* tmem_slot = reinterpret_cast<uint32_t*>(tile_empty + 2);
   int* s_n = reinterpret_cast<int*>(tmem_slot + 1);
+  int* s_item = s_n + 2;
 
   const int warp = threadIdx.x >> 5, lane = threadIdx.x & 31;
-  const int kv0 = blockIdx.x * kT, h = blockIdx.y, b = blockIdx.z;
   const int nqb = p.S / kT;
   if (warp == 0) TRACE(5, 63);
   if (warp == kDrainWarp0 && lane == 0) {
     tma_prefetch_desc(&tmQ);
     tma_prefetch_desc(&tmDO);
     tma_prefetch_desc(&tmDQ);
-    tma_prefetch_desc(&tmDK);
-    tma_prefetch_desc(&tmDV);
+    tma_prefetch_desc(&tmK);
+    tma_prefetch_desc(&tmV);
   }
   if (warp == kBwdTmaWarp && lane == 0) {
     mbar_init(kv_full, 1);
-    fence_mbar_init();
-    mbar_expect_tx(kv_full, 2 * BwdSmem::kTile);
-    tma_load_2d(sK, &tmK, kv_full, h * kD, b * p.Nk + kv0);
-    tma_load_2d(sV, &tmV, kv_full, h * kD, b * p.Nk + kv0);
     for (int i = 0; i < kBwdStages; ++i) { mbar_init(&q_full[i], 1); mbar_init(&q_empty[i], 1); }
     mbar_init(s_full, 1);   mbar_init(s_free, kBwdMathWarps);
     mbar_init(dp_full, 1);  mbar_init(dp_free, 1);
     mbar_init(p_full, kBwdMathWarps);  mbar_init(p_empty, 1);
     mbar_init(ds_full, kBwdMathWarps); mbar_init(ds_empty, 1);
     mbar_init(dq_full, 1);  mbar_init(dq_free, 4);
-    mbar_init(dkv_full, 1);
+    mbar_init(dkv_full, 1); mbar_init(dkv_free, 4);
     mbar_init(kv_tmem, kBwdMathWarps);
+    mbar_init(&k_free[0], 1); mbar_init(&k_free[1], 1);
+    mbar_init(v_free, kBwdMathWarps);
+    for (int i = 0; i < 2; ++i) { mbar_init(&tile_full[i], 1); mbar_init(&tile_empty[i], kBwdMathWarps + 6); }
     fence_mbar_init();
-    TRACE(5, 57);
-  }
-  auto issue_q_block = [&](int qblk, int st) {
-    const int r0 = qblk * kT;
-    uint8_t* meta = sMeta + st * kBwdMetaBytes;
-    const int64_t hoff = ((int64_t)b * p.H + h) * p.S + r0, roff = (int64_t)b * p.S + r0;
-    mbar_expect_tx(&q_full[st], 2 * BwdSmem::kTile + kBwdMetaBytes);
-    tma_load_2d(sQ + st * BwdSmem::kTile, &tmQ, &q_full[st], h * kD, b * p.Mq + r0);
-    tma_load_2d(sDO + st * BwdSmem::kTile, &tmDO, &q_full[st], h * kD, b * p.Mq + r0);
-    bulk_load(meta + 0 * 512, p.lse2 + hoff, 512, &q_full[st]);
-    bulk_load(meta + 1 * 512, p.ndelta + hoff, 512, &q_full[st]);
-    bulk_load(meta + 2 * 512, p.meta.row_lo + roff, 512, &q_full[st]);
-    bulk_load(meta + 3 * 512, p.meta.row_hi + roff, 512, &q_full[st]);
-    bulk_load(meta + 4 * 512, p.meta.row_scale + roff, 512, &q_full[st]);
-  };
-  if (warp == kBwdTmaWarp) {
-    int first = -1;
-    for (int i0 = 0; i0 < nqb && first < 0; i0 += 32) {
-      const int i = i0 + lane;
-      bool take = false;
-      if (i < nqb) {
-        const int64_t o = ((int64_t)b * nqb + i) * 2;
-        const int lo = min(p.meta.blk_lo[o], p.meta.blk_lo[o + 1]), hi = max(p.meta.blk_hi[o], p.meta.blk_hi[o + 1]);
-        take = hi > kv0 && lo < kv0 + kT;
-      }
-      const unsigned msk = __ballot_sync(0xffffffffu, take);
-      if (msk) first = i0 + __ffs(msk) - 1;
-    }
-    __syncwarp();
-    if (first >= 0 && lane == 0) issue_q_block(first, 0);
-  }
-  if (warp == 0) {
-    int n = 0;
-    for (int i0 = 0; i0 < nqb; i0 += 32) {
-      const int i = i0 + lane;
-      bool take = false, inside = false, normal = false;
-      if (i < nqb) {
-        const int64_t o = ((int64_t)b * nqb + i) * 2;
-        const int lo = min(p.meta.blk_lo[o], p.meta.blk_lo[o + 1]), hi = max(p.meta.blk_hi[o], p.meta.blk_hi[o + 1]);
-        take = hi > kv0 && lo < kv0 + kT;
-        inside = max(p.meta.blk_lo_max[o], p.meta.blk_lo_max[o + 1]) <= kv0 &&
-                 min(p.meta.blk_hi_min[o], p.meta.blk_hi_min[o + 1]) >= kv0 + kT;
-        normal = p.meta.blk_lo_max[o] != INT_MAX && p.meta.blk_lo_max[o + 1] != INT_MAX;
-      }
-      const unsigned msk = __ballot_sync(0xffffffffu, take);
-      const int pos = n + __popc(msk & ((1u << lane) - 1));
-      if (take && pos < kMaxQBlocks) s_list[pos] = (uint16_t)(i | (inside ? 0x8000 : 0) | (normal ? 0x4000 : 0));
-      n += __popc(msk);
-    }
-    if (lane == 0) *s_n = n < kMaxQBlocks ? n : kMaxQBlocks;
-    TRACE(5, 55);
   }
   if (warp == kBwdMmaWarp) {
     tmem_alloc<512>(tmem_slot);
     TRACE(5, 54);
   }
-  if (warp == 1) TRACE(5, 53);
   tc_fence_before();
   __syncthreads();
   tc_fence_after();
   const uint32_t tmem_base = *tmem_slot;
-  const int n = *s_n;
   if (warp == 0) TRACE(5, 62);
   constexpr uint32_t cS = 0, cDP = 128, cDV = 256, cDK = 320, cDQ = 384, cK = 448, cV = 480;
 
+  auto decode = [&](int item, int& kv0, int& h, int& b) {
+    const int bh = item / p.ntiles;
+    kv0 = (item - bh * p.ntiles) * kT;
+    h = bh % p.H;
+    b = bh / p.H;
+  };
+  auto take_tile = [&](int it) {
+    mbar_wait(&tile_full[it & 1], (it >> 1) & 1);
+    return s_n[it & 1];
+  };
+  auto release_tile = [&](int it) {
+    __syncwarp();
+    if (lane == 0) mbar_arrive(&tile_empty[it & 1]);
+  };
+
   if (warp >= kBwdTmaWarp) {
     if (warp == kBwdTmaWarp) {
-      if (n == 0) mbar_wait(kv_full, 0);
-      if (n > 0) {
-        for (int idx = 1; idx < n; ++idx) {
-          const int st = idx % kBwdStages;
-          mbar_wait(&q_empty[st], ((idx / kBwdStages) & 1) ^ 1);
-          if (elect_one()) issue_q_block((int)(s_list[idx] & 0x3fff), st);
+      int g = 0, kvt = 0;
+      unsigned item = bwd_claim_item(p.counter);
+      for (int it = 0;; ++it) {
+        const int buf = it & 1;
+        mbar_wait(&tile_empty[buf], ((it >> 1) & 1) ^ 1);
+        if (item >= (unsigned)p.items) {
+          if (lane == 0) {
+            s_n[buf] = -1;
+            mbar_arrive(&tile_full[buf]);
+          }
+          break;
+        }
+        int kv0, h, b;
+        decode((int)item, kv0, h, b);
+        uint16_t* list = s_list + buf * kMaxQBlocks;
+        int n = 0;
+        for (int i0 = 0; i0 < nqb; i0 += 32) {
+          const int i = i0 + lane;
+          bool take = false, inside = false, normal = false;
+          if (i < nqb) {
+            const int64_t o = ((int64_t)b * nqb + i) * 2;
+            const int lo = min(p.meta.blk_lo[o], p.meta.blk_lo[o + 1]), hi = max(p.meta.blk_hi[o], p.meta.blk_hi[o + 1]);
+            take = hi > kv0 && lo < kv0 + kT;
+            inside = max(p.meta.blk_lo_max[o], p.meta.blk_lo_max[o + 1]) <= kv0 &&
+                     min(p.meta.blk_hi_min[o], p.meta.blk_hi_min[o + 1]) >= kv0 + kT;
+            normal = p.meta.blk_lo_max[o] != INT_MAX && p.meta.blk_lo_max[o + 1] != INT_MAX;
+          }
+          const unsigned msk = __ballot_sync(0xffffffffu, take);
+          const int pos = n + __popc(msk & ((1u << lane) - 1));
+          if (take && pos < kMaxQBlocks) list[pos] = (uint16_t)(i | (inside ? 0x8000 : 0) | (normal ? 0x4000 : 0));
+          n += __popc(msk);
+        }
+        n = min(n, kMaxQBlocks);
+        if (lane == 0) {
+          s_n[buf] = n;
+          s_item[buf] = (int)item;
+        }
+        __threadfence_block();
+        __syncwarp();
+        if (lane == 0) mbar_arrive(&tile_full[buf]);
+        item = bwd_claim_item(p.counter);
+        if (n > 0) {
+          const int slot = kvt & 1;
+          mbar_wait(&k_free[slot], ((kvt >> 1) & 1) ^ 1);
+          mbar_wait(v_free, (kvt & 1) ^ 1);
+          if (lane == 0) {
+            mbar_expect_tx(kv_full, 2 * BwdSmem::kTile);
+            tma_load_2d(sK + slot * BwdSmem::kTile, &tmK, kv_full, h * kD, b * p.Nk + kv0);
+            tma_load_2d(sV, &tmV, kv_full, h * kD, b * p.Nk + kv0);
+          }
           __syncwarp();
+          for (int j = 0; j < n; ++j, ++g) {
+            const int st = g % kBwdStages;
+            mbar_wait(&q_empty[st], ((g / kBwdStages) & 1) ^ 1);
+            if (elect_one()) {
+              const int r0 = (int)(list[j] & 0x3fff) * kT;
+              uint8_t* meta = sMeta + st * kBwdMetaBytes;
+              const int64_t hoff = ((int64_t)b * p.H + h) * p.S + r0, roff = (int64_t)b * p.S + r0;
+              mbar_expect_tx(&q_full[st], 2 * BwdSmem::kTile + kBwdMetaBytes);
+              tma_load_2d(sQ + st * BwdSmem::kTile, &tmQ, &q_full[st], h * kD, b * p.Mq + r0);
+              tma_load_2d(sDO + st * BwdSmem::kTile, &tmDO, &q_full[st], h * kD, b * p.Mq + r0);
+              bulk_load(meta + 0 * 512, p.lse2 + hoff, 512, &q_full[st]);
+              bulk_load(meta + 1 * 512, p.ndelta + hoff, 512, &q_full[st]);
+              bulk_load(meta + 2 * 512, p.meta.row_lo + roff, 512, &q_full[st]);
+              bulk_load(meta + 3 * 512, p.meta.row_hi + roff, 512, &q_full[st]);
+              bulk_load(meta + 4 * 512, p.meta.row_scale + roff, 512, &q_full[st]);
+            }
+            __syncwarp();
+          }
+          ++kvt;
         }
       }
     } else if (warp == kBwdMmaWarp) {
-      if (n > 0) {
-        constexpr uint32_t idesc_kk = umma_idesc_bf16(128, kT, 0, 0);
-        constexpr uint32_t idesc_tm = umma_idesc_bf16(128, kD, 0, 1);
-        constexpr uint32_t idesc_mm = umma_idesc_bf16(128, kD, 1, 1);
-        const uint32_t tS = tmem_base + cS, tDP = tmem_base + cDP, tDQ = tmem_base + cDQ, tK = tmem_base + cK, tV = tmem_base + cV;
-        const uint64_t dKm0 = umma_desc_mnmajor_sw128(smem_u32(sK), 8192);
-        const uint64_t dDSm0 = umma_desc_mnmajor_sw128(smem_u32(sDS), BwdSmem::kTile);
-        auto issue_s = [&](int st) {
-          const uint64_t dQ0 = umma_desc_kmajor_sw128(smem_u32(sQ + st * BwdSmem::kTile));
-          if (elect_one()) {
-#pragma unroll
-            for (int k = 0; k < 4; ++k) umma_bf16_ts(tS, tK + 8 * k, dQ0 + 2 * k, idesc_kk, k ? 1u : 0u);
-            umma_commit(s_full);
-          }
-          __syncwarp();
-        };
-        auto issue_dp = [&](int st) {
-          const uint64_t dDO0 = umma_desc_kmajor_sw128(smem_u32(sDO + st * BwdSmem::kTile));
-          if (elect_one()) {
-#pragma unroll
-            for (int k = 0; k < 4; ++k) umma_bf16_ts(tDP, tV + 8 * k, dDO0 + 2 * k, idesc_kk, k ? 1u : 0u);
-            umma_commit(dp_full);
-          }
-          __syncwarp();
-        };
-        mbar_wait(kv_tmem, 0);
-        mbar_wait(&q_full[0], 0);
-        tc_fence_after();
-        issue_s(0);
-        issue_dp(0);
-        for (int idx = 0; idx < n; ++idx) {
-          const int st1 = (idx + 1) % kBwdStages;
-          const uint32_t par = idx & 1;
-          if (idx + 1 < n) {
-            mbar_wait(&q_full[st1], ((idx + 1) / kBwdStages) & 1);
+      constexpr uint32_t idesc_kk = umma_idesc_bf16(128, kT, 0, 0);
+      constexpr uint32_t idesc_mm = umma_idesc_bf16(128, kD, 1, 1);
+      const uint32_t tS = tmem_base + cS, tDP = tmem_base + cDP, tDQ = tmem_base + cDQ, tK = tmem_base + cK, tV = tmem_base + cV;
+      const uint64_t dDSm0 = umma_desc_mnmajor_sw128(smem_u32(sDS), BwdSmem::kTile);
+      auto issue_s = [&](int st) {
+        const uint64_t dQ0 = umma_desc_kmajor_sw128(smem_u32(sQ + st * BwdSmem::kTile));
+        if (elect_one()) {
+#pragma unroll
+          for (int k = 0; k < 4; ++k) umma_bf16_ts(tS, tK + 8 * k, dQ0 + 2 * k, idesc_kk, k ? 1u : 0u);
+          umma_commit(s_full);
+        }
+        __syncwarp();
+      };
+      auto issue_dp = [&](int st) {
+        const uint64_t dDO0 = umma_desc_kmajor_sw128(smem_u32(sDO + st * BwdSmem::kTile));
+        if (elect_one()) {
+#pragma unroll
+          for (int k = 0; k < 4; ++k) umma_bf16_ts(tDP, tV + 8 * k, dDO0 + 2 * k, idesc_kk, k ? 1u : 0u);
+          umma_commit(dp_full);
+        }
+        __syncwarp();
+      };
+      int g = 0, kvt = 0;
+      bool pre = false;
+      for (int it = 0;; ++it) {
+        const int n = take_tile(it);
+        release_tile(it);
+        if (n < 0) break;
+        if (n == 0) continue;
+        const int slot = kvt & 1;
+        const uint64_t dKm0 = umma_desc_mnmajor_sw128(smem_u32(sK + slot * BwdSmem::kTile), 8192);
+        if (!pre) {
+          mbar_wait(kv_tmem, kvt & 1);
+          mbar_wait(&q_full[g % kBwdStages], (g / kBwdStages) & 1);
+          if (g > 0) {
+            mbar_wait(s_free, (g - 1) & 1);
+            mbar_wait(p_empty, (g - 1) & 1);
+          }
+          tc_fence_after();
+          TRACE_B(0, g);
+          issue_s(g % kBwdStages);
+          if (g > 0) {
+            mbar_wait(dp_free, (g - 1) & 1);
+            tc_fence_after();
+          }
+          issue_dp(g % kBwdStages);
+        }
+        pre = false;
+        for (int j = 0; j < n; ++j, ++g) {
+          const int st1 = (g + 1) % kBwdStages;
+          const uint32_t par = g & 1;
+          bool next = j + 1 < n;
+          if (!next && take_tile(it + 1) > 0) {
+            mbar_wait(kv_tmem, (kvt + 1) & 1);
+            next = pre = true;
+          }
+          if (next) {
+            mbar_wait(&q_full[st1], ((g + 1) / kBwdStages) & 1);
             mbar_wait(s_free, par);
             mbar_wait(p_empty, par);
             tc_fence_after();
-            TRACE(0, idx);
+            TRACE_B(0, g + 1);
             issue_s(st1);
           }
           mbar_wait(ds_full, par);
-          if (idx > 0) mbar_wait(dq_free, (idx - 1) & 1);
+          if (g > 0) mbar_wait(dq_free, (g - 1) & 1);
           tc_fence_after();
-          TRACE(4, idx);
+          TRACE_B(4, g);
           if (elect_one()) {
 #pragma unroll
             for (int k = 0; k < 8; ++k) umma_bf16_ss(tDQ, dDSm0 + 128 * k, dKm0 + 128 * k, idesc_mm, k ? 1u : 0u);
             umma_commit(dq_full);
             umma_commit(ds_empty);
+            if (j + 1 == n) umma_commit(&k_free[slot]);
           }
           __syncwarp();
-          if (idx + 1 < n) {
+          if (next) {
             mbar_wait(dp_free, par);
             tc_fence_after();
-            TRACE(2, idx);
+            TRACE_B(2, g + 1);
             issue_dp(st1);
           }
         }
+        ++kvt;
       }
     } else if (warp == kBwdMmaWarpB) {
-      if (n > 0) {
-        constexpr uint32_t idesc_tm = umma_idesc_bf16(128, kD, 0, 1);
-        const uint32_t tS = tmem_base + cS, tDP = tmem_base + cDP, tDV = tmem_base + cDV, tDK = tmem_base + cDK;
-        for (int idx = 0; idx < n; ++idx) {
-          const int st = idx % kBwdStages;
-          const uint32_t par = idx & 1;
+      constexpr uint32_t idesc_tm = umma_idesc_bf16(128, kD, 0, 1);
+      const uint32_t tS = tmem_base + cS, tDP = tmem_base + cDP, tDV = tmem_base + cDV, tDK = tmem_base + cDK;
+      int g = 0, kvt = 0;
+      for (int it = 0;; ++it) {
+        const int n = take_tile(it);
+        release_tile(it);
+        if (n < 0) break;
+        if (n == 0) continue;
+        for (int j = 0; j < n; ++j, ++g) {
+          const int st = g % kBwdStages;
+          const uint32_t par = g & 1;
           mbar_wait(p_full, par);
+          if (j == 0) mbar_wait(dkv_free, (kvt & 1) ^ 1);
           tc_fence_after();
-          TRACE(1, idx);
+          TRACE_B(1, g);
           const uint64_t dDOm0 = umma_desc_mnmajor_sw128(smem_u32(sDO + st * BwdSmem::kTile), 8192);
           if (elect_one()) {
 #pragma unroll
             for (int k = 0; k < 8; ++k)
-              umma_bf16_ts(tDV, tS + (k < 4 ? 8 * k : 64 + 8 * (k - 4)), dDOm0 + 128 * k, idesc_tm, (idx | k) ? 1u : 0u);
+              umma_bf16_ts(tDV, tS + (k < 4 ? 8 * k : 64 + 8 * (k - 4)), dDOm0 + 128 * k, idesc_tm, (j | k) ? 1u : 0u);
             umma_commit(p_empty);
           }
           __syncwarp();
           mbar_wait(ds_full, par);
           tc_fence_after();
-          TRACE(3, idx);
+          TRACE_B(3, g);
           const uint64_t dQm0 = umma_desc_mnmajor_sw128(smem_u32(sQ + st * BwdSmem::kTile), 8192);
           if (elect_one()) {
 #pragma unroll
             for (int k = 0; k < 8; ++k)
-              umma_bf16_ts(tDK, tDP + (k < 4 ? 8 * k : 64 + 8 * (k - 4)), dQm0 + 128 * k, idesc_tm, (idx | k) ? 1u : 0u);
+              umma_bf16_ts(tDK, tDP + (k < 4 ? 8 * k : 64 + 8 * (k - 4)), dQm0 + 128 * k, idesc_tm, (j | k) ? 1u : 0u);
             umma_commit(&q_empty[st]);
             umma_commit(dp_free);
-            if (idx == n - 1) umma_commit(dkv_full);
+            if (j + 1 == n) umma_commit(dkv_full);
           }
           __syncwarp();
         }
+        ++kvt;
       }
     }
   } else if (warp >= kDrainWarp0) {
     const int quarter = warp & 3;
     uint8_t* box0 = sBox + quarter * 8192;
-    const uint32_t t_dq = tmem_base + ((uint32_t)(quarter * 32) << 16) + cDQ;
-    for (int idx = 0; idx < n; ++idx) {
-      const int r0 = (int)(s_list[idx] & 0x3fff) * kT + quarter * 32;
-      mbar_wait(dq_full, idx & 1);
-      tc_fence_after();
-      if (warp == kDrainWarp0) TRACE(11, idx);
-      const bool live = r0 < p.Mq;
+    const uint32_t t_q = tmem_base + ((uint32_t)(quarter * 32) << 16);
+    int g = 0, kvt = 0;
+    for (int it = 0;; ++it) {
+      const int n = take_tile(it);
+      if (n < 0) break;
+      int kv0, h, b;
+      decode(s_item[it & 1], kv0, h, b);
+      const uint16_t* list = s_list + (it & 1) * kMaxQBlocks;
+      for (int j = 0; j < n; ++j, ++g) {
+        const int r0 = (int)(list[j] & 0x3fff) * kT + quarter * 32;
+        mbar_wait(dq_full, g & 1);
+        tc_fence_after();
+        if (warp == kDrainWarp0) TRACE_B(11, g);
+        const bool live = r0 < p.Mq;
+        if (lane == 0) tma_store_wait_read();
+        __syncwarp();
+#pragma unroll
+        for (int hb = 0; hb < 2; ++hb) {
+          uint32_t v[32];
+          uint8_t* box = box0 + hb * 4096;
+          tmem_ld32(t_q + cDQ + hb * 32, v);
+          tmem_ld_wait();
+          if (hb == 1) {
+            tc_fence_before();
+            __syncwarp();
+            if (lane == 0) mbar_arrive(dq_free);
+          }
+          if (live) {
+#pragma unroll
+            for (int j8 = 0; j8 < 8; ++j8)
+              *reinterpret_cast<uint4*>(box + lane * 128 + ((j8 ^ (lane & 7)) << 4)) = make_uint4(v[4 * j8], v[4 * j8 + 1], v[4 * j8 + 2], v[4 * j8 + 3]);
+            fence_async_smem();
+            __syncwarp();
+            if (lane == 0) {
+              tma_reduce_add_2d(&tmDQ, box, h * kD + hb * 32, b * p.Mq + r0);
+              tma_store_commit();
+            }
+          }
+        }
+        if (warp == kDrainWarp0) TRACE_B(12, g);
+      }
+      release_tile(it);
+      if (n > 0) {
+        mbar_wait(dkv_full, kvt & 1);
+        tc_fence_after();
+      }
       if (lane == 0) tma_store_wait_read();
       __syncwarp();
 #pragma unroll
-      for (int hb = 0; hb < 2; ++hb) {
-        uint32_t v[32];
-        uint8_t* box = box0 + hb * 4096;
-        tmem_ld32(t_dq + hb * 32, v);
-        tmem_ld_wait();
-        if (hb == 1) {
-          tc_fence_before();
-          __syncwarp();
-          if (lane == 0) mbar_arrive(dq_free);
-        }
-        if (live) {
-#pragma unroll
-          for (int j = 0; j < 8; ++j)
-            *reinterpret_cast<uint4*>(box + lane * 128 + ((j ^ (lane & 7)) << 4)) = make_uint4(v[4 * j], v[4 * j + 1], v[4 * j + 2], v[4 * j + 3]);
-          fence_async_smem();
-          __syncwarp();
-          if (lane == 0) {
-            tma_reduce_add_2d(&tmDQ, box, h * kD + hb * 32, b * p.Mq + r0);
-            tma_store_commit();
-          }
-        }
-      }
-      if (warp == kDrainWarp0) TRACE(12, idx);
+      for (int which = 0; which < 2; ++which) {
+        uint8_t* box = box0 + which * 4096;
+#pragma unroll
+        for (int hb = 0; hb < 2; ++hb) {
+          uint32_t v[32];
+          if (n > 0) {
+            tmem_ld32(t_q + (which == 0 ? cDV : cDK) + hb * 32, v);
+            tmem_ld_wait();
+          } else {
+#pragma unroll
+            for (int c = 0; c < 32; ++c) v[c] = 0u;
+          }
+#pragma unroll
+          for (int c8 = 0; c8 < 4; ++c8)
+            *reinterpret_cast<uint4*>(box + lane * 128 + (((hb * 4 + c8) ^ (lane & 7)) << 4)) =
+                make_uint4(pack_bf16(__uint_as_float(v[c8 * 8 + 0]), __uint_as_float(v[c8 * 8 + 1])),
+                           pack_bf16(__uint_as_float(v[c8 * 8 + 2]), __uint_as_float(v[c8 * 8 + 3])),
+                           pack_bf16(__uint_as_float(v[c8 * 8 + 4]), __uint_as_float(v[c8 * 8 + 5])),
+                           pack_bf16(__uint_as_float(v[c8 * 8 + 6]), __uint_as_float(v[c8 * 8 + 7])));
+        }
+      }
+      if (n > 0) {
+        tc_fence_before();
+        __syncwarp();
+        if (lane == 0) mbar_arrive(dkv_free);
+        ++kvt;
+      }
+      __syncwarp();
+#pragma unroll
+      for (int which = 0; which < 2; ++which) {
+        const uint8_t* box = box0 + which * 4096;
+        uint16_t* base = which == 0 ? p.dV : p.dK;
+        const int64_t ld = which == 0 ? p.lddv : p.lddk;
+#pragma unroll
+        for (int i = 0; i < 8; ++i) {
+          const int row = i * 4 + (lane >> 3), chunk = lane & 7;
+          const int key = kv0 + quarter * 32 + row;
+          const uint4 val = *reinterpret_cast<const uint4*>(box + row * 128 + ((chunk ^ (row & 7)) << 4));
+          if (key < p.Nk) reinterpret_cast<uint4*>(base + ((int64_t)b * p.Nk + key) * ld + h * kD)[chunk] = val;
+        }
+      }
+      __syncwarp();
+      if (warp == kDrainWarp0 && kvt <= 4) TRACE(5, 47 + kvt);
     }
     if (lane == 0) tma_store_wait_read();
   } else {
     const int quarter = warp & 3, half = warp >> 2;
     const int trow = quarter * 32 + lane;
-    const int kidx = kv0 + trow;
     const uint32_t t_lane = tmem_base + ((uint32_t)(quarter * 32) << 16);
     uint8_t* pDS = sDS + half * BwdSmem::kTile;
     const float SC = p.scale_log2, RN = p.scale_log2 * kLn2;
-    if (n > 0) {
-      mbar_wait(kv_full, 0);
-      if (warp == 0) TRACE(5, 56);
-      uint32_t kw[16], vw[16];
-#pragma unroll
-      for (int c = 0; c < 4; ++c) {
-        const uint4 a = *reinterpret_cast<const uint4*>(sK + swz_off(trow, half * 4 + c));
-        const uint4 d = *reinterpret_cast<const uint4*>(sV + swz_off(trow, half * 4 + c));
-        kw[4 * c] = a.x; kw[4 * c + 1] = a.y; kw[4 * c + 2] = a.z; kw[4 * c + 3] = a.w;
-        vw[4 * c] = d.x; vw[4 * c + 1] = d.y; vw[4 * c + 2] = d.z; vw[4 * c + 3] = d.w;
-      }
-      tmem_st16(t_lane + cK + half * 16, kw);
-      tmem_st16(t_lane + cV + half * 16, vw);
+    auto copy_kv = [&](int kt) {
+      mbar_wait(kv_full, kt & 1);
+      const uint8_t* k_s = sK + (kt & 1) * BwdSmem::kTile;
+#pragma unroll
+      for (int which = 0; which < 2; ++which) {
+        const uint8_t* src = which == 0 ? k_s : sV;
+        uint32_t w[16];
+#pragma unroll
+        for (int c = 0; c < 4; ++c) {
+          const uint4 a = *reinterpret_cast<const uint4*>(src + swz_off(trow, half * 4 + c));
+          w[4 * c] = a.x; w[4 * c + 1] = a.y; w[4 * c + 2] = a.z; w[4 * c + 3] = a.w;
+        }
+        tmem_st16(t_lane + (which == 0 ? cK : cV) + half * 16, w);
+      }
       tmem_st_wait();
       tc_fence_before();
       __syncwarp();
-      if (lane == 0) mbar_arrive(kv_tmem);
-      if (warp == 0) TRACE(5, 58);
-    }
-    for (int idx = 0; idx < n; ++idx) {
-      const int st = idx % kBwdStages;
-      const uint32_t par = idx & 1;
-      const bool inside = (s_list[idx] & 0x8000) != 0, normal = (s_list[idx] & 0x4000) != 0;
-      const float* m_ls = reinterpret_cast<const float*>(sMeta + st * kBwdMetaBytes) + half * 64;
-      const float* m_nd = m_ls + kT;
-      const int* m_lo = reinterpret_cast<const int*>(m_ls + 2 * kT);
-      const int* m_hi = m_lo + kT;
-      const float* m_rs = m_ls + 4 * kT;
-      uint32_t pp[32];
-      {
-        uint32_t s0[32], s1[32];
-        if (warp == 0) TRACE(5, idx);
-        mbar_wait(&q_full[st], (idx / kBwdStages) & 1);
-        mbar_wait(s_full, par);
+      if (lane == 0) {
+        mbar_arrive(v_free);
+        mbar_arrive(kv_tmem);
+      }
+    };
+    int g = 0, kvt = 0;
+    bool pre = false;
+    for (int it = 0;; ++it) {
+      const int n = take_tile(it);
+      if (n <= 0) {
+        release_tile(it);
+        if (n < 0) break;
+        continue;
+      }
+      const int kidx = (s_item[it & 1] % p.ntiles) * kT + trow;
+      const uint16_t* list = s_list + (it & 1) * kMaxQBlocks;
+      if (!pre) copy_kv(kvt);
+      pre = false;
+      for (int j = 0; j < n; ++j, ++g) {
+        const int st = g % kBwdStages;
+        const uint32_t par = g & 1;
+        const bool inside = (list[j] & 0x8000) != 0, normal = (list[j] & 0x4000) != 0;
+        const float* m_ls = reinterpret_cast<const float*>(sMeta + st * kBwdMetaBytes) + half * 64;
+        const float* m_nd = m_ls + kT;
+        const int* m_lo = reinterpret_cast<const int*>(m_ls + 2 * kT);
+        const int* m_hi = m_lo + kT;
+        const float* m_rs = m_ls + 4 * kT;
+        uint32_t pp[32];
+        {
+          uint32_t s0[32], s1[32];
+          if (warp == 0) TRACE_B(5, g);
+          mbar_wait(&q_full[st], (g / kBwdStages) & 1);
+          mbar_wait(s_full, par);
+          tc_fence_after();
+          if (warp == 0) TRACE_B(6, g);
+          tmem_ld32(t_lane + cS + half * 64, s0);
+          tmem_ld32(t_lane + cS + half * 64 + 32, s1);
+          tmem_ld_wait();
+          tc_fence_before();
+          __syncwarp();
+          if (lane == 0) mbar_arrive(s_free);
+          if (inside) {
+#pragma unroll
+            for (int c4 = 0; c4 < 8; ++c4) {
+              const float4 la = lds_f4(m_ls + 4 * c4), lb = lds_f4(m_ls + 32 + 4 * c4);
+              s0[4 * c4] = __float_as_uint(fmaf(__uint_as_float(s0[4 * c4]), SC, -la.x));
+              s0[4 * c4 + 1] = __float_as_uint(fmaf(__uint_as_float(s0[4 * c4 + 1]), SC, -la.y));
+              s0[4 * c4 + 2] = __float_as_uint(fmaf(__uint_as_float(s0[4 * c4 + 2]), SC, -la.z));
+              s0[4 * c4 + 3] = __float_as_uint(fmaf(__uint_as_float(s0[4 * c4 + 3]), SC, -la.w));
+              s1[4 * c4] = __float_as_uint(fmaf(__uint_as_float(s1[4 * c4]), SC, -lb.x));
+              s1[4 * c4 + 1] = __float_as_uint(fmaf(__uint_as_float(s1[4 * c4 + 1]), SC, -lb.y));
+              s1[4 * c4 + 2] = __float_as_uint(fmaf(__uint_as_float(s1[4 * c4 + 2]), SC, -lb.z));
+              s1[4 * c4 + 3] = __float_as_uint(fmaf(__uint_as_float(s1[4 * c4 + 3]), SC, -lb.w));
+            }
+#pragma unroll
+            for (int c = 0; c < 32; ++c) {
+              s0[c] = __float_as_uint((c & 3) == 3 ? ex2_poly(__uint_as_float(s0[c])) : ex2(__uint_as_float(s0[c])));
+              s1[c] = __float_as_uint((c & 3) == 3 ? ex2_poly(__uint_as_float(s1[c])) : ex2(__uint_as_float(s1[c])));
+            }
+#pragma unroll
+            for (int c = 0; c < 16; ++c) {
+              pp[c] = pack_bf16(__uint_as_float(s0[2 * c]), __uint_as_float(s0[2 * c + 1]));
+              pp[16 + c] = pack_bf16(__uint_as_float(s1[2 * c]), __uint_as_float(s1[2 * c + 1]));
+            }
+          } else if (normal) {
+#pragma unroll
+            for (int c4 = 0; c4 < 8; ++c4) {
+#pragma unroll
+              for (int g = 0; g < 2; ++g) {
+                uint32_t(&sv)[32] = g ? s1 : s0;
+                const float4 l = lds_f4(m_ls + g * 32 + 4 * c4), lo = lds_f4(m_lo + g * 32 + 4 * c4), hi = lds_f4(m_hi + g * 32 + 4 * c4);
+                const float lv[4] = {l.x, l.y, l.z, l.w};
+                const int lov[4] = {__float_as_int(lo.x), __float_as_int(lo.y), __float_as_int(lo.z), __float_as_int(lo.w)};
+                const int hiv[4] = {__float_as_int(hi.x), __float_as_int(hi.y), __float_as_int(hi.z), __float_as_int(hi.w)};
+#pragma unroll
+                for (int u = 0; u < 4; ++u) {
+                  const bool ok = kidx >= lov[u] && kidx < hiv[u];
+                  sv[4 * c4 + u] = ok ? __float_as_uint(fmaf(__uint_as_float(sv[4 * c4 + u]), SC, -lv[u])) : 0xff800000u;
+                }
+              }
+            }
+#pragma unroll
+            for (int c = 0; c < 32; ++c) {
+              s0[c] = __float_as_uint(ex2(__uint_as_float(s0[c])));
+              s1[c] = __float_as_uint(ex2(__uint_as_float(s1[c])));
+            }
+#pragma unroll
+            for (int c = 0; c < 16; ++c) {
+              pp[c] = pack_bf16(__uint_as_float(s0[2 * c]), __uint_as_float(s0[2 * c + 1]));
+              pp[16 + c] = pack_bf16(__uint_as_float(s1[2 * c]), __uint_as_float(s1[2 * c + 1]));
+            }
+          } else {
+#pragma unroll
+            for (int c = 0; c < 32; ++c) {
+              float e[2];
+#pragma unroll
+              for (int u = 0; u < 2; ++u) {
+                const int q = 2 * c + u;
+                const float rs = m_rs[q];
+                const bool ok = kidx >= m_lo[q] && kidx < m_hi[q];
+                const float sv = __uint_as_float(q < 32 ? s0[q & 31] : s1[q & 31]);
+                e[u] = ok ? ex2(fmaf(rs != 0.f ? sv : 0.f, rs, -m_ls[q])) : 0.f;
+              }
+              pp[c] = pack_bf16(e[0], e[1]);
+            }
+          }
+        }
+        if (warp == 0) TRACE_B(7, g);
+        tmem_st32(t_lane + cS + half * 64, pp);
+        uint32_t d0[32];
+        mbar_wait(dp_full, par);
         tc_fence_after();
-        if (warp == 0) TRACE(6, idx);
-        tmem_ld32(t_lane + cS + half * 64, s0);
-        tmem_ld32(t_lane + cS + half * 64 + 32, s1);
-        tmem_ld_wait();
+        tmem_ld32(t_lane + cDP + half * 64, d0);
+        tmem_st_wait();
         tc_fence_before();
         __syncwarp();
-        if (lane == 0) mbar_arrive(s_free);
-        if (inside) {
-#pragma unroll
-          for (int c4 = 0; c4 < 8; ++c4) {
-            const float4 la = lds_f4(m_ls + 4 * c4), lb = lds_f4(m_ls + 32 + 4 * c4);
-            s0[4 * c4] = __float_as_uint(fmaf(__uint_as_float(s0[4 * c4]), SC, -la.x));
-            s0[4 * c4 + 1] = __float_as_uint(fmaf(__uint_as_float(s0[4 * c4 + 1]), SC, -la.y));
-            s0[4 * c4 + 2] = __float_as_uint(fmaf(__uint_as_float(s0[4 * c4 + 2]), SC, -la.z));
-            s0[4 * c4 + 3] = __float_as_uint(fmaf(__uint_as_float(s0[4 * c4 + 3]), SC, -la.w));
-            s1[4 * c4] = __float_as_uint(fmaf(__uint_as_float(s1[4 * c4]), SC, -lb.x));
-            s1[4 * c4 + 1] = __float_as_uint(fmaf(__uint_as_float(s1[4 * c4 + 1]), SC, -lb.y));
-            s1[4 * c4 + 2] = __float_as_uint(fmaf(__uint_as_float(s1[4 * c4 + 2]), SC, -lb.z));
-            s1[4 * c4 + 3] = __float_as_uint(fmaf(__uint_as_float(s1[4 * c4 + 3]), SC, -lb.w));
-          }
-#pragma unroll
-          for (int c = 0; c < 32; ++c) {
-            s0[c] = __float_as_uint((c & 3) == 3 ? ex2_poly(__uint_as_float(s0[c])) : ex2(__uint_as_float(s0[c])));
-            s1[c] = __float_as_uint((c & 3) == 3 ? ex2_poly(__uint_as_float(s1[c])) : ex2(__uint_as_float(s1[c])));
-          }
-#pragma unroll
-          for (int c = 0; c < 16; ++c) {
-            pp[c] = pack_bf16(__uint_as_float(s0[2 * c]), __uint_as_float(s0[2 * c + 1]));
-            pp[16 + c] = pack_bf16(__uint_as_float(s1[2 * c]), __uint_as_float(s1[2 * c + 1]));
-          }
-        } else if (normal) {
-#pragma unroll
-          for (int c4 = 0; c4 < 8; ++c4) {
-#pragma unroll
-            for (int g = 0; g < 2; ++g) {
-              uint32_t(&sv)[32] = g ? s1 : s0;
-              const float4 l = lds_f4(m_ls + g * 32 + 4 * c4), lo = lds_f4(m_lo + g * 32 + 4 * c4), hi = lds_f4(m_hi + g * 32 + 4 * c4);
-              const float lv[4] = {l.x, l.y, l.z, l.w};
-              const int lov[4] = {__float_as_int(lo.x), __float_as_int(lo.y), __float_as_int(lo.z), __float_as_int(lo.w)};
-              const int hiv[4] = {__float_as_int(hi.x), __float_as_int(hi.y), __float_as_int(hi.z), __float_as_int(hi.w)};
-#pragma unroll
-              for (int u = 0; u < 4; ++u) {
-                const bool ok = kidx >= lov[u] && kidx < hiv[u];
-                sv[4 * c4 + u] = ok ? __float_as_uint(fmaf(__uint_as_float(sv[4 * c4 + u]), SC, -lv[u])) : 0xff800000u;
-              }
-            }
-          }
-#pragma unroll
-          for (int c = 0; c < 32; ++c) {
-            s0[c] = __float_as_uint(ex2(__uint_as_float(s0[c])));
-            s1[c] = __float_as_uint(ex2(__uint_as_float(s1[c])));
-          }
-#pragma unroll
-          for (int c = 0; c < 16; ++c) {
-            pp[c] = pack_bf16(__uint_as_float(s0[2 * c]), __uint_as_float(s0[2 * c + 1]));
-            pp[16 + c] = pack_bf16(__uint_as_float(s1[2 * c]), __uint_as_float(s1[2 * c + 1]));
-          }
-        } else {
-#pragma unroll
-          for (int c = 0; c < 32; ++c) {
-            float e[2];
-#pragma unroll
-            for (int u = 0; u < 2; ++u) {
-              const int q = 2 * c + u;
-              const float rs = m_rs[q];
-              const bool ok = kidx >= m_lo[q] && kidx < m_hi[q];
-              const float sv = __uint_as_float(q < 32 ? s0[q & 31] : s1[q & 31]);
-              e[u] = ok ? ex2(fmaf(rs != 0.f ? sv : 0.f, rs, -m_ls[q])) : 0.f;
-            }
-            pp[c] = pack_bf16(e[0], e[1]);
-          }
-        }
-      }
-      if (warp == 0) TRACE(7, idx);
-      tmem_st32(t_lane + cS + half * 64, pp);
-      uint32_t d0[32];
-      mbar_wait(dp_full, par);
-      tc_fence_after();
-      tmem_ld32(t_lane + cDP + half * 64, d0);
-      tmem_st_wait();
-      tc_fence_before();
-      __syncwarp();
-      if (lane == 0) mbar_arrive(p_full);
-      if (warp == 0) TRACE(8, idx);
-      auto dsmul = [&](const uint32_t (&d)[32], int hh) {
-        if (inside || normal) {
-#pragma unroll
-          for (int c4 = 0; c4 < 8; ++c4) {
-            const float4 nd = lds_f4(m_nd + hh * 32 + 4 * c4);
-            const uint32_t t0 = pack_bf16(fmaf(__uint_as_float(d[4 * c4]), RN, nd.x), fmaf(__uint_as_float(d[4 * c4 + 1]), RN, nd.y));
-            const uint32_t t1 = pack_bf16(fmaf(__uint_as_float(d[4 * c4 + 2]), RN, nd.z), fmaf(__uint_as_float(d[4 * c4 + 3]), RN, nd.w));
-            asm("mul.rn.bf16x2 %0, %1, %2;" : "=r"(pp[hh * 16 + 2 * c4]) : "r"(pp[hh * 16 + 2 * c4]), "r"(t0));
-            asm("mul.rn.bf16x2 %0, %1, %2;" : "=r"(pp[hh * 16 + 2 * c4 + 1]) : "r"(pp[hh * 16 + 2 * c4 + 1]), "r"(t1));
-          }
-        } else {
-#pragma unroll
-          for (int c4 = 0; c4 < 8; ++c4) {
-            const float4 nd = lds_f4(m_nd + hh * 32 + 4 * c4);
-            const float4 rs = lds_f4(m_rs + hh * 32 + 4 * c4);
-            const uint32_t t0 = pack_bf16(fmaf(__uint_as_float(d[4 * c4]), rs.x * kLn2, nd.x), fmaf(__uint_as_float(d[4 * c4 + 1]), rs.y * kLn2, nd.y));
-            const uint32_t t1 = pack_bf16(fmaf(__uint_as_float(d[4 * c4 + 2]), rs.z * kLn2, nd.z), fmaf(__uint_as_float(d[4 * c4 + 3]), rs.w * kLn2, nd.w));
-            asm("mul.rn.bf16x2 %0, %1, %2;" : "=r"(pp[hh * 16 + 2 * c4]) : "r"(pp[hh * 16 + 2 * c4]), "r"(t0));
-            asm("mul.rn.bf16x2 %0, %1, %2;" : "=r"(pp[hh * 16 + 2 * c4 + 1]) : "r"(pp[hh * 16 + 2 * c4 + 1]), "r"(t1));
-          }
-        }
-      };
-      tmem_ld_wait();
-      if (warp == 0) TRACE(9, idx);
-      dsmul(d0, 0);
-      if (warp == 0) TRACE(13, idx);
-      tmem_ld32(t_lane + cDP + half * 64 + 32, d0);
-      if (idx > 0) mbar_wait(ds_empty, (idx - 1) & 1);
-      tmem_ld_wait();
-      if (warp == 0) TRACE(14, idx);
-      dsmul(d0, 1);
-      if (warp == 0) TRACE(15, idx);
-      tmem_st32(t_lane + cDP + half * 64, pp);
-#pragma unroll
-      for (int c8 = 0; c8 < 8; ++c8)
-        *reinterpret_cast<uint4*>(pDS + swz_off(trow, c8)) = make_uint4(pp[4 * c8], pp[4 * c8 + 1], pp[4 * c8 + 2], pp[4 * c8 + 3]);
-      fence_async_smem();
-      tmem_st_wait();
-      tc_fence_before();
-      __syncwarp();
-      if (lane == 0) mbar_arrive(ds_full);
-      if (warp == 0) TRACE(10, idx);
+        if (lane == 0) mbar_arrive(p_full);
+        if (warp == 0) TRACE_B(8, g);
+        auto dsmul = [&](const uint32_t (&d)[32], int hh) {
+          if (inside || normal) {
+#pragma unroll
+            for (int c4 = 0; c4 < 8; ++c4) {
+              const float4 nd = lds_f4(m_nd + hh * 32 + 4 * c4);
+              const uint32_t t0 = pack_bf16(fmaf(__uint_as_float(d[4 * c4]), RN, nd.x), fmaf(__uint_as_float(d[4 * c4 + 1]), RN, nd.y));
+              const uint32_t t1 = pack_bf16(fmaf(__uint_as_float(d[4 * c4 + 2]), RN, nd.z), fmaf(__uint_as_float(d[4 * c4 + 3]), RN, nd.w));
+              asm("mul.rn.bf16x2 %0, %1, %2;" : "=r"(pp[hh * 16 + 2 * c4]) : "r"(pp[hh * 16 + 2 * c4]), "r"(t0));
+              asm("mul.rn.bf16x2 %0, %1, %2;" : "=r"(pp[hh * 16 + 2 * c4 + 1]) : "r"(pp[hh * 16 + 2 * c4 + 1]), "r"(t1));
+            }
+          } else {
+#pragma unroll
+            for (int c4 = 0; c4 < 8; ++c4) {
+              const float4 nd = lds_f4(m_nd + hh * 32 + 4 * c4);
+              const float4 rs = lds_f4(m_rs + hh * 32 + 4 * c4);
+              const uint32_t t0 = pack_bf16(fmaf(__uint_as_float(d[4 * c4]), rs.x * kLn2, nd.x), fmaf(__uint_as_float(d[4 * c4 + 1]), rs.y * kLn2, nd.y));
+              const uint32_t t1 = pack_bf16(fmaf(__uint_as_float(d[4 * c4 + 2]), rs.z * kLn2, nd.z), fmaf(__uint_as_float(d[4 * c4 + 3]), rs.w * kLn2, nd.w));
+              asm("mul.rn.bf16x2 %0, %1, %2;" : "=r"(pp[hh * 16 + 2 * c4]) : "r"(pp[hh * 16 + 2 * c4]), "r"(t0));
+              asm("mul.rn.bf16x2 %0, %1, %2;" : "=r"(pp[hh * 16 + 2 * c4 + 1]) : "r"(pp[hh * 16 + 2 * c4 + 1]), "r"(t1));
+            }
+          }
+        };
+        tmem_ld_wait();
+        if (warp == 0) TRACE_B(9, g);
+        dsmul(d0, 0);
+        if (warp == 0) TRACE_B(13, g);
+        if (j + 1 == n && take_tile(it + 1) > 0) {
+          copy_kv(kvt + 1);
+          pre = true;
+        }
+        tmem_ld32(t_lane + cDP + half * 64 + 32, d0);
+        if (g > 0) mbar_wait(ds_empty, (g - 1) & 1);
+        tmem_ld_wait();
+        if (warp == 0) TRACE_B(14, g);
+        dsmul(d0, 1);
+        if (warp == 0) TRACE_B(15, g);
+        tmem_st32(t_lane + cDP + half * 64, pp);
+#pragma unroll
+        for (int c8 = 0; c8 < 8; ++c8)
+          *reinterpret_cast<uint4*>(pDS + swz_off(trow, c8)) = make_uint4(pp[4 * c8], pp[4 * c8 + 1], pp[4 * c8 + 2], pp[4 * c8 + 3]);
+        fence_async_smem();
+        tmem_st_wait();
+        tc_fence_before();
+        __syncwarp();
+        if (lane == 0) mbar_arrive(ds_full);
+        if (warp == 0) TRACE_B(10, g);
+      }
+      release_tile(it);
+      ++kvt;
     }
-    if (n > 0) {
-      mbar_wait(dkv_full, 0);
-      tc_fence_after();
-    }
-    if (warp == 0) TRACE(5, 61);
-#pragma unroll 1
-    for (int which = 0; which < 2; ++which) {
-      uint32_t v[32];
-      if (n > 0) {
-        tmem_ld32(t_lane + (which == 0 ? cDV : cDK) + half * 32, v);
-        tmem_ld_wait();
-      } else {
-#pragma unroll
-        for (int c = 0; c < 32; ++c) v[c] = 0u;
-      }
-      uint4 pk[4];
-#pragma unroll
-      for (int c8 = 0; c8 < 4; ++c8) {
-        pk[c8].x = pack_bf16(__uint_as_float(v[c8 * 8 + 0]), __uint_as_float(v[c8 * 8 + 1]));
-        pk[c8].y = pack_bf16(__uint_as_float(v[c8 * 8 + 2]), __uint_as_float(v[c8 * 8 + 3]));
-        pk[c8].z = pack_bf16(__uint_as_float(v[c8 * 8 + 4]), __uint_as_float(v[c8 * 8 + 5]));
-        pk[c8].w = pack_bf16(__uint_as_float(v[c8 * 8 + 6]), __uint_as_float(v[c8 * 8 + 7]));
-      }
-      if (p.tma_out) {
-        uint8_t* stage = which == 0 ? sQ : sDO;
-#pragma unroll
-        for (int c8 = 0; c8 < 4; ++c8) *reinterpret_cast<uint4*>(stage + swz_off(trow, half * 4 + c8)) = pk[c8];
-        if (warp == 0) TRACE(5, 52 - which);
-      } else if (kidx < p.Nk) {
-        uint16_t* out = (which == 0 ? p.dV + ((int64_t)b * p.Nk + kidx) * p.lddv : p.dK + ((int64_t)b * p.Nk + kidx) * p.lddk) +
-                        h * kD + half * 32;
-#pragma unroll
-        for (int c8 = 0; c8 < 4; ++c8) reinterpret_cast<uint4*>(out)[c8] = pk[c8];
-      }
-    }
-    if (p.tma_out) {
-      fence_async_smem();
-      asm volatile("bar.sync 1, 256;" ::: "memory");
-      if (warp == 0) TRACE(5, 50);
-      if (warp == 0 && lane == 0) {
-        tma_store_2d(&tmDV, sQ, h * kD, b * p.Nk + kv0);
-        tma_store_2d(&tmDK, sDO, h * kD, b * p.Nk + kv0);
-        tma_store_commit();
-        tma_store_wait_read();
-      }
-    }
-    if (warp == 0) TRACE(5, 60);
   }
   tc_fence_before();
   __syncthreads();
@@ -561,7 +665,9 @@
 
 __global__ void __launch_bounds__(256) attn_bwd_prep_kernel(const uint16_t* __restrict__ O, const uint16_t* __restrict__ dO,
                                                             int64_t ldo, const float* __restrict__ row_scale, int B, int H,
-                                                            int Mq, int S, float* __restrict__ ndelta, float* __restrict__ dq_acc) {
+                                                            int Mq, int S, float* __restrict__ ndelta, float* __restrict__ dq_acc,
+                                                            unsigned* __restrict__ counter) {
+  if (blockIdx.x == 0 && threadIdx.x == 0) *counter = 0u;
   const int64_t wid = (int64_t)blockIdx.x * 8 + (threadIdx.x >> 5);
   const int lane = threadIdx.x & 31;
   if (wid >= (int64_t)B * S) return;
@@ -621,16 +727,18 @@
 
 extern "C" int64_t egom2p_attn_bwd_scratch_bytes(int32_t B, int32_t H, int32_t Mq) {
   using namespace egom2p;
-  return align256((int64_t)B * H * padS(Mq) * 4) + align256((int64_t)B * Mq * H * kD * 4) + 256;
+  return align256((int64_t)B * H * padS(Mq) * 4) + align256((int64_t)B * Mq * H * kD * 4) + 256 + 256;
 }
 
 extern "C" int egom2p_attn_bwd(const uint16_t* Q, const uint16_t* K, const uint16_t* V, const uint16_t* O, const uint16_t* dO,
                                const float* lse, int32_t B, int32_t H, int32_t Mq, int32_t Nk, int64_t ldq, int64_t ldk,
                                int64_t ldv, int64_t ldo, const void* meta, float scale, void* scratch, uint16_t* dQ,
-                               uint16_t* dK, uint16_t* dV, int64_t lddq, int64_t lddk, int64_t lddv, void* stream_) {
+                               uint16_t* dK, uint16_t* dV, int64_t lddq, int64_t lddk, int64_t lddv, void* stream_,
+                               int32_t ctas) {
   using namespace egom2p;
   cudaStream_t stream = (cudaStream_t)stream_;
-  EGO_REQUIRE(Q && O && dO && lse && meta && scratch && dQ && B > 0 && H > 0 && Mq > 0 && Nk >= 0, "attn_bwd: bad argument");
+  EGO_REQUIRE(Q && O && dO && lse && meta && scratch && dQ && B > 0 && H > 0 && Mq > 0 && Nk >= 0 && ctas >= 0,
+              "attn_bwd: bad argument");
   EGO_REQUIRE(((uintptr_t)scratch & 255) == 0 && ((uintptr_t)lse & 255) == 0 && ((uintptr_t)meta & 255) == 0,
               "attn_bwd: scratch / lse / meta must be 256-byte aligned");
   EGO_REQUIRE(lddq % 8 == 0 && ((uintptr_t)dQ & 15) == 0 && ldo % 8 == 0 && ((uintptr_t)O & 15) == 0 && ((uintptr_t)dO & 15) == 0,
@@ -640,8 +748,10 @@
   RangeMeta rm = carve_meta(const_cast<void*>(meta), B, Mq);
   float* ndelta = reinterpret_cast<float*>(scratch);
   float* dq_acc = reinterpret_cast<float*>(reinterpret_cast<char*>(scratch) + align256((int64_t)B * H * S * 4));
-
-  attn_bwd_prep_kernel<<<(unsigned)(((int64_t)B * S + 7) / 8), 256, 0, stream>>>(O, dO, ldo, rm.row_scale, B, H, Mq, S, ndelta, dq_acc);
+  unsigned* counter = reinterpret_cast<unsigned*>(reinterpret_cast<char*>(dq_acc) + align256((int64_t)B * Mq * H * kD * 4));
+
+  attn_bwd_prep_kernel<<<(unsigned)(((int64_t)B * S + 7) / 8), 256, 0, stream>>>(O, dO, ldo, rm.row_scale, B, H, Mq, S, ndelta, dq_acc,
+                                                                                 counter);
   int rc = check_launch("attn_bwd prep");
   if (rc) return rc;
   if (Nk > 0) {
@@ -649,22 +759,18 @@
     EGO_REQUIRE(lddk % 8 == 0 && lddv % 8 == 0 && ((uintptr_t)dK & 15) == 0 && ((uintptr_t)dV & 15) == 0, "attn_bwd: dK/dV alignment");
     static std::atomic<uint64_t> attr_done{0};
     if ((rc = ensure_dyn_smem(attn_bwd_kernel, BwdSmem::kTotal, attr_done, "attn_bwd"))) return rc;
-    CUtensorMap tmQ, tmDO, tmK, tmV, tmDQ, tmDK, tmDV;
+    CUtensorMap tmQ, tmDO, tmK, tmV, tmDQ;
     if ((rc = make_tmap_bf16_2d(&tmQ, Q, (uint64_t)B * Mq, (uint64_t)H * kD, ldq, kT, kD))) return rc;
     if ((rc = make_tmap_bf16_2d(&tmDO, dO, (uint64_t)B * Mq, (uint64_t)H * kD, ldo, kT, kD))) return rc;
     if ((rc = make_tmap_bf16_2d(&tmK, K, (uint64_t)B * Nk, (uint64_t)H * kD, ldk, kT, kD))) return rc;
     if ((rc = make_tmap_bf16_2d(&tmV, V, (uint64_t)B * Nk, (uint64_t)H * kD, ldv, kT, kD))) return rc;
     if ((rc = make_tmap_2d(&tmDQ, dq_acc, 4, (uint64_t)B * Mq, (uint64_t)H * kD, (uint64_t)H * kD, 32, 32))) return rc;
-    const int tma_out = (Nk % kT == 0 || B == 1) ? 1 : 0;
-    if (tma_out) {
-      if ((rc = make_tmap_bf16_2d(&tmDK, dK, (uint64_t)B * Nk, (uint64_t)H * kD, lddk, kT, kD))) return rc;
-      if ((rc = make_tmap_bf16_2d(&tmDV, dV, (uint64_t)B * Nk, (uint64_t)H * kD, lddv, kT, kD))) return rc;
-    } else {
-      tmDK = tmK;
-      tmDV = tmV;
-    }
-    BwdParams pb{B, H, Mq, Nk, S, rm, lse, ndelta, scale * kLog2e, dK, dV, lddk, lddv, tma_out};
-    attn_bwd_kernel<<<dim3((Nk + kT - 1) / kT, H, B), kBwdThreads, BwdSmem::kTotal, stream>>>(tmQ, tmDO, tmK, tmV, tmDQ, tmDK, tmDV, pb);
+    const int ntiles = (Nk + kT - 1) / kT;
+    const int64_t items = (int64_t)B * H * ntiles;
+    EGO_REQUIRE(items <= INT_MAX, "attn_bwd: too many key tiles");
+    const int64_t grid = std::min<int64_t>(ctas > 0 ? ctas : device_sm_count(), items);
+    BwdParams pb{B, H, Mq, Nk, S, ntiles, (int)items, counter, rm, lse, ndelta, scale * kLog2e, dK, dV, lddk, lddv};
+    attn_bwd_kernel<<<(unsigned)grid, kBwdThreads, BwdSmem::kTotal, stream>>>(tmQ, tmDO, tmK, tmV, tmDQ, pb);
     if ((rc = check_launch("attn_bwd"))) return rc;
   }
   const int64_t rows = (int64_t)B * Mq;
diff --git a/egom2p_b200/ops.py b/egom2p_b200/ops.py
--- a/egom2p_b200/ops.py
+++ b/egom2p_b200/ops.py
@@ -360,7 +360,8 @@
     return o, lse
 
 
-def attn_bwd(q, k, v, o, do, lse, B, H, Mq, Nk, dq, dk, dv, key_lo=None, key_hi=None, scale=None, meta=None, pairs=None):
+def attn_bwd(q, k, v, o, do, lse, B, H, Mq, Nk, dq, dk, dv, key_lo=None, key_hi=None, scale=None, meta=None, pairs=None,
+             ctas=0):
     lib = _lib.load()
     scale = (64 ** -0.5) if scale is None else scale
     if meta is None:
@@ -370,7 +371,7 @@
     with _timed("attn_bwd", 10.0 * H * 64 * (pairs if pairs is not None else B * Mq * Nk), "flop"):
         _lib.check(lib.egom2p_attn_bwd(_p(q), _p(k), _p(v), _p(o), _p(do), _p(lse), B, H, Mq, Nk, q.stride(0), k.stride(0),
                                        v.stride(0), o.stride(0), _p(meta), scale, _p(scratch), _p(dq), _p(dk), _p(dv),
-                                       dq.stride(0), dk.stride(0), dv.stride(0), _s()), "attn_bwd")
+                                       dq.stride(0), dk.stride(0), dv.stride(0), _s(), ctas), "attn_bwd")
 
 
 def cast_bf16(src: torch.Tensor, out: Optional[torch.Tensor] = None):
diff --git a/include/egom2p_b200.h b/include/egom2p_b200.h
--- a/include/egom2p_b200.h
+++ b/include/egom2p_b200.h
@@ -99,7 +99,7 @@
 int egom2p_attn_bwd(const uint16_t* Q, const uint16_t* K, const uint16_t* V, const uint16_t* O, const uint16_t* dO,
                     const float* lse, int32_t B, int32_t H, int32_t Mq, int32_t Nk, int64_t ldq, int64_t ldk, int64_t ldv,
                     int64_t ldo, const void* meta, float scale, void* scratch, uint16_t* dQ, uint16_t* dK, uint16_t* dV,
-                    int64_t lddq, int64_t lddk, int64_t lddv, void* stream);
+                    int64_t lddq, int64_t lddk, int64_t lddv, void* stream, int32_t ctas);
 
 int egom2p_cast_f32_to_bf16(const float* src, uint16_t* dst, int64_t n, void* stream);
 typedef struct {
```

Result: no change. 707,700, median of 6 (+0.2%).
